# peterropac/Aegolius

Hardware: AMD Instinct MI355X
Metric: Mpoints/sec SDF eval, 1024^3 grid, 10-prim smooth-union tree (higher is better)
Workload: dtype f32

## Files before the change

aegolius_amd/_engine.py:

```python
import atexit
import contextlib
import ctypes
import importlib.util
import os
import sys
import threading

import numpy as np

_HERE = os.path.dirname(os.path.abspath(__file__))
LIB_PATH = os.path.join(_HERE, "libsdfk.so")

MODE_AUTO, MODE_INTERPRET, MODE_SPECIALIZED, MODE_NOCULL = 0, 1, 2, 3
(FLAVOUR_PLAIN_ARRAY, FLAVOUR_PLAIN_GRID, FLAVOUR_TILE_ARRAY, FLAVOUR_TILE_GRID, FLAVOUR_TILE_MASK, FLAVOUR_ROWS_ARRAY,
 FLAVOUR_ROWS_GRID, FLAVOUR_ROWS_MASK, FLAVOUR_ROWS2D_ARRAY, FLAVOUR_ROWS2D_GRID, FLAVOUR_RAYS) = range(11)
FLAVOUR_FLAGS = 0x100
FLAVOUR_XY = 0x200

_c = ctypes
_vp, _i64, _int, _sz = _c.c_void_p, _c.c_int64, _c.c_int, _c.c_size_t
_fp = _c.POINTER(_c.c_float)

SIGNATURES = {
    "sdfk_abi_version": (_int, []),
    "sdfk_device_count": (_int, []),
    "sdfk_last_error": (_c.c_char_p, []),
    "sdfk_program_create": (_vp, [_vp, _sz, _vp, _sz, _vp, _sz, _int]),
    "sdfk_program_destroy": (None, [_vp]),
    "sdfk_program_set_params": (_int, [_vp, _vp, _sz]),
    "sdfk_program_set_cull": (_int, [_vp, _vp, _sz, _vp]),
    "sdfk_program_source": (_c.c_char_p, [_vp]),
    "sdfk_program_compile_check": (_int, [_vp, _c.POINTER(_sz)]),
    "sdfk_program_chain_members": (_int, [_vp]),
    "sdfk_program_compile_flavour": (_int, [_vp, _int, _c.POINTER(_sz), _c.POINTER(_c.c_double)]),
    "sdfk_debug_compile_external": (_int, [_vp, _int, _c.POINTER(_sz)]),
    "sdfk_debug_jit_stats": (None, [_c.POINTER(_i64), _c.POINTER(_c.c_double)]),
    "sdfk_jit_drain": (None, []),
    "sdfk_jit_cancel": (None, []),
    "sdfk_debug_set_rtc_defs": (None, [_c.c_char_p]),
    "sdfk_eval_device": (_int, [_vp, _vp, _i64, _i64, _vp, _vp, _int]),
    "sdfk_eval_device_rows": (_int, [_vp, _vp, _i64, _i64, _i64, _vp, _vp, _int]),
    "sdfk_eval_device_rows2d": (_int, [_vp, _vp, _i64, _i64, _i64, _vp, _vp, _int]),
    "sdfk_eval_device_rows2d_xy": (_int, [_vp, _vp, _i64, _i64, _i64, _vp, _vp, _int]),
    "sdfk_debug_cells_stats": (None, [_int, _c.POINTER(_c.c_longlong)]),
    "sdfk_debug_rays_stats": (None, [_int, _c.POINTER(_c.c_longlong)]),
    "sdfk_eval_device_rows3d": (_int, [_vp, _vp, _i64, _i64, _i64, _i64, _i64, _vp, _vp, _int]),
    "sdfk_debug_row_masks": (_int, [_vp, _vp, _i64, _i64, _i64, _vp, _c.POINTER(_i64), _c.POINTER(_int), _vp]),
    "sdfk_eval_grid_sharded": (_int, [_vp, _vp, _i64, _vp, _i64, _vp, _i64, _int, _vp, _vp, _int]),
    "sdfk_eval_grid_sharded_device": (_int, [_vp, _vp, _i64, _vp, _i64, _vp, _i64, _int, _vp, _int, _vp, _int]),
    "sdfk_eval_device_aux": (_int, [_vp, _vp, _i64, _i64, _vp, _int, _i64, _vp, _vp, _int]),
    "sdfk_eval_grid_aux": (_int, [_vp, _vp, _i64, _vp, _i64, _vp, _i64, _i64, _i64, _vp, _int, _i64, _vp, _vp, _int]),
    "sdfk_field_min": (_int, [_vp, _i64, _c.POINTER(_c.c_float), _vp]),
    "sdfk_grid_box_average": (_int, [_vp, _i64, _i64, _i64, _int, _int, _int, _int, _vp, _vp]),
    "sdfk_grid_edge_detect": (_int, [_vp, _i64, _i64, _i64, _vp, _vp]),
    "sdfk_grid_signed": (_int, [_vp, _i64, _i64, _i64, _c.c_float, _int, _vp, _vp]),
    "sdfk_grid_boundary_mask": (_int, [_vp, _i64, _c.c_float, _vp, _vp]),
    "sdfk_grid_signed_slab": (_int, [_vp, _i64, _i64, _vp, _i64, _i64, _i64, _int, _vp, _vp]),
    "sdfk_eval_host": (_int, [_vp, _vp, _int, _i64, _i64, _vp, _int, _int]),
    "sdfk_eval_host_resident": (_int, [_vp, _vp, _int, _i64, _i64, _vp, _int, _int]),
    "sdfk_field_select_scratch": (_sz, [_i64]),
    "sdfk_field_select": (_int, [_vp, _i64, _c.c_float, _vp, _i64, _c.POINTER(_i64), _vp, _vp]),
    "sdfk_field_select_finish": (_int, [_i64, _i64, _vp, _i64, _vp, _vp]),
    "sdfk_field_gradient": (_int, [_vp, _i64, _i64, _i64, _int, _int, _vp, _i64, _vp]),
    "sdfk_field_crossings_2d": (_int, [_vp, _vp, _i64, _i64, _i64, _c.c_double, _c.c_double, _c.c_double, _vp, _vp]),
    "sdfk_lcwg_eval": (_int, [_int, _vp, _vp, _i64, _i64, _i64, _c.c_double, _c.c_double, _int, _c.c_double, _vp, _vp, _i64,
                              _vp]),
    "sdfk_lcwg_old_eval": (_int, [_int, _vp, _i64, _vp, _i64, _c.c_double, _c.c_double, _vp, _i64, _vp]),
    "sdfk_eval_select_scratch": (_sz, [_i64, _i64]),
    "sdfk_eval_device_select": (_int, [_vp, _vp, _i64, _i64, _i64, _int, _c.c_float, _vp, _i64, _c.POINTER(_i64), _vp, _vp, _int]),
    "sdfk_eval_grid_select": (_int, [_vp, _vp, _i64, _vp, _i64, _vp, _i64, _i64, _i64, _c.c_float, _vp, _i64, _c.POINTER(_i64),
                                     _vp, _vp, _int]),
    "sdfk_eval_select_finish": (_int, [_vp, _i64, _i64, _int, _i64, _vp, _i64, _vp, _vp]),
    "sdfk_vec_eval_device": (_int, [_vp, _int, _vp, _i64, _i64, _vp, _int, _i64, _int, _vp, _i64, _vp]),
    "sdfk_vec_set_interpret": (None, [_int]),
    "sdfk_vec_source": (_c.c_char_p, [_vp, _int, _int, _int]),
    "sdfk_vec_compile_check": (_int, [_vp, _int, _int, _int, _c.POINTER(_sz)]),
    "sdfk_vec_eval_host": (_int, [_vp, _int, _vp, _int, _i64, _vp, _i64, _vp, _i64, _vp, _i64, _vp, _int, _int, _vp, _int]),
    "sdfk_eval_grid": (_int, [_vp, _vp, _i64, _vp, _i64, _vp, _i64, _i64, _i64, _vp, _vp, _int]),
    "sdfk_eval_grid_host": (_int, [_vp, _vp, _i64, _vp, _i64, _vp, _i64, _i64, _i64, _vp, _int, _int]),
    "sdfk_set_default_mode": (None, [_int]),
    "sdfk_debug_brick_masks": (_int, [_vp, _vp, _i64, _i64, _vp, _vp]),
    "sdfk_linspace_f32": (_int, [_c.c_double, _c.c_double, _i64, _vp]),
    "sdfk_point_tree_build": (_i64, [_vp, _i64, _int, _vp, _i64, _vp, _vp, _vp]),
    "sdfk_grid_fill": (_int, [_vp, _i64, _vp, _i64, _vp, _i64, _vp, _i64, _i64, _i64, _vp]),
    "sdfk_set_device": (_int, [_int]),
    "sdfk_malloc": (_vp, [_sz]),
    "sdfk_free": (_int, [_vp]),
    "sdfk_memcpy_h2d": (_int, [_vp, _vp, _sz]),
    "sdfk_memcpy_d2h": (_int, [_vp, _vp, _sz]),
    "sdfk_memcpy_d2d": (_int, [_vp, _vp, _sz]),
    "sdfk_sync": (_int, [_vp]),
    "sdfk_event_create": (_vp, []),
    "sdfk_event_destroy": (_int, [_vp]),
    "sdfk_event_record": (_int, [_vp, _vp]),
    "sdfk_event_elapsed_ms": (_int, [_vp, _vp, _fp]),
    "sdfk_stream_probe": (_int, [_vp, _i64, _i64, _vp, _vp]),
    "sdfk_dual_has_rule": (_int, [_int]),
    "sdfk_program_jvp_check": (_int, [_vp, _c.POINTER(_int)]),
    "sdfk_eval_jvp_device": (_int, [_vp, _vp, _i64, _i64, _vp, _int, _int, _vp, _vp, _i64, _vp]),
    "sdfk_value_jvp_device": (_int, [_int, _vp, _vp, _vp, _i64, _vp, _vp, _vp]),
    "sdfk_program_vjp_check": (_int, [_vp, _c.POINTER(_int), _c.POINTER(_i64)]),
    "sdfk_vjp_limits": (_int, [_c.POINTER(_int), _c.POINTER(_int)]),
    "sdfk_eval_vjp_device": (_int, [_vp, _vp, _i64, _i64, _vp, _int, _int, _vp, _vp, _vp, _vp]),
    "sdfk_points_bin": (_int, [_vp, _i64, _i64, _vp, _i64, _i64, _i64, _vp, _vp]),
    "sdfk_points_extent": (_int, [_vp, _i64, _i64, _i64, _vp, _vp]),
    "sdfk_points_fill": (_int, [_vp, _i64, _i64, _i64, _int, _i64, _i64, _i64, _vp]),
    "sdfk_points_widen": (_int, [_vp, _i64, _int, _vp, _vp]),
    "sdfk_field_isosurface_scratch": (_sz, [_i64, _i64, _i64]),
    "sdfk_field_isosurface": (_int, [_vp, _vp, _i64, _vp, _i64, _vp, _i64, _c.c_float, _c.POINTER(_i64), _c.POINTER(_i64), _vp,
                                     _vp]),
    "sdfk_field_isosurface_finish": (_int, [_vp, _i64, _i64, _i64, _c.c_float, _i64, _i64, _vp, _i64, _vp, _i64, _int, _vp,
                                            _vp]),
    "sdfk_field_contour2d_scratch": (_sz, [_i64, _i64]),
    "sdfk_field_contour2d": (_int, [_vp, _vp, _i64, _vp, _i64, _c.c_float, _c.POINTER(_i64), _c.POINTER(_i64), _vp, _vp]),
    "sdfk_field_contour2d_finish": (_int, [_vp, _i64, _i64, _c.c_float, _i64, _i64, _vp, _i64, _vp, _i64, _int, _vp, _vp]),
    "sdfk_eval_grid_isosurface_scratch": (_sz, [_i64, _i64, _i64]),
    "sdfk_eval_grid_isosurface": (_int, [_vp, _vp, _i64, _vp, _i64, _vp, _i64, _c.c_float, _c.POINTER(_i64), _c.POINTER(_i64),
                                         _vp, _vp, _int]),
    "sdfk_eval_grid_isosurface_finish": (_int, [_vp, _vp, _i64, _vp, _i64, _vp, _i64, _c.c_float, _i64, _i64, _vp, _i64, _vp,
                                                _i64, _int, _vp, _vp, _int]),
    "sdfk_eval_grid_contour2d_scratch": (_sz, [_i64, _i64]),
    "sdfk_eval_grid_contour2d": (_int, [_vp, _vp, _i64, _vp, _i64, _c.c_float, _c.POINTER(_i64), _c.POINTER(_i64), _vp, _vp,
# ... 168 lines not shown

    def _filled(self, fill, *args):
        try:
            fill(*args)
        except BaseException:
            self.free()
            raise
        return self

    def free(self):
        _release(self, "ptr", "sdfk_free")

    def __enter__(self):
        return self

    def __exit__(self, *exc):
        self.free()

    def __del__(self):
        self.free()


class DeviceRows(DeviceBuffer):

    def __init__(self, rows, n, device=None, what=""):
        self.rows, self.n, self.stride = int(rows), int(n), row_stride(int(n))
        DeviceBuffer.__init__(self, self.rows * self.stride * 4, device, what)

    def offset(self, r):
        return 4 * r * self.stride

    def row(self, r):
        return self.at(self.offset(r), 4 * self.n)

    def row_ptr(self, r):
        return self.row(r).value

    def upload_rows(self, host):
        for r, line in enumerate(np.ascontiguousarray(host, dtype=np.float32)):
            self.upload(line, self.offset(r))

    def download_rows(self, count=None):
        out = np.empty((self.rows if count is None else count, self.n), dtype=np.float32)
        for r, line in enumerate(out):
            self.download(line, self.offset(r))
        return out


class Program:

    def __init__(self, code, params, tables, result_reg, cull_sites=None, cull_k=None):
        self.code = np.ascontiguousarray(code, dtype=np.uint32).reshape(-1, 2)
        self.params = np.ascontiguousarray(params, dtype=np.float32).ravel()
        self.tables = np.ascontiguousarray(tables, dtype=np.float32).ravel()
        self.result_reg = int(result_reg)
        self._h = lib().sdfk_program_create(_ptr(self.code), self.code.shape[0], _ptr(self.params), self.params.size,
                                            _ptr(self.tables), self.tables.size, self.result_reg)
        if not self._h:
            raise SdfkError("sdfk_program_create rejected the program: " + last_error())
        if cull_sites is not None and len(cull_sites):
            sites = np.ascontiguousarray(cull_sites, dtype=np.uint32).reshape(-1, 5)
            k = np.ascontiguousarray(cull_k, dtype=np.float32).ravel()
            check(lib().sdfk_program_set_cull(self._h, _ptr(sites), sites.shape[0], _ptr(k)), "sdfk_program_set_cull")

    @classmethod
    def from_lowered(cls, low, cull=True):
        if cull:
            return cls(low.code, low.params, low.tables, low.result_reg, low.cull_sites, low.cull_k)
        return cls(low.code, low.params, low.tables, low.result_reg)

    @property
    def handle(self):
        return self._h

    def set_params(self, params):
        p = np.ascontiguousarray(params, dtype=np.float32).ravel()
        check(lib().sdfk_program_set_params(self._h, _ptr(p), p.size), "sdfk_program_set_params")
        self.params = p

    def source(self):
        s = lib().sdfk_program_source(self._h)
        return s.decode() if s else None

    @property
    def chain_members(self):
        return int(lib().sdfk_program_chain_members(self._h))

    def compile_check(self):
        n = _sz(0)
        check(lib().sdfk_program_compile_check(self._h, ctypes.byref(n)), "sdfk_program_compile_check")
        return n.value

    def compile_flavour(self, flavour):
        n, t = _sz(0), _c.c_double(0.0)
        check(lib().sdfk_program_compile_flavour(self._h, int(flavour), ctypes.byref(n), ctypes.byref(t)),
              "sdfk_program_compile_flavour")
        return n.value, t.value

    def eval_host(self, co, device=0, mode=MODE_AUTO):
        require_gpu()
        co = host_coords(co)
        n = co.shape[1]
        out = np.empty(n, dtype=np.float32)
        check(lib().sdfk_eval_host(self._h, _ptr(co), 0 if co.dtype == np.float32 else 1, n, n, _ptr(out), device,
                                   mode), "sdfk_eval_host")
        return out

    def eval_device(self, d_co, n, row_stride, d_out, stream=None, mode=MODE_AUTO, row_len=None, flat=False,
                    plane_rows=None, first_row_in_plane=0):
        if row_len and plane_rows and not flat:
            check(lib().sdfk_eval_device_rows3d(self._h, _vp(d_co), n, row_stride, int(row_len), int(plane_rows),
                                                int(first_row_in_plane), _vp(d_out), _vp(stream or 0), mode),
                  "sdfk_eval_device_rows3d")
            return
        if row_len and flat:
            check(lib().sdfk_eval_device_rows2d(self._h, _vp(d_co), n, row_stride, int(row_len), _vp(d_out),
                                                _vp(stream or 0), mode), "sdfk_eval_device_rows2d")
            return
        if row_len:
            check(lib().sdfk_eval_device_rows(self._h, _vp(d_co), n, row_stride, int(row_len), _vp(d_out),
                                              _vp(stream or 0), mode), "sdfk_eval_device_rows")
            return
        check(lib().sdfk_eval_device(self._h, _vp(d_co), n, row_stride, _vp(d_out), _vp(stream or 0), mode),
              "sdfk_eval_device")

    def eval_device_xy(self, d_xy, n, row_stride, d_out, stream=None, mode=MODE_AUTO, row_len=None):
        check(lib().sdfk_eval_device_rows2d_xy(self._h, _vp(d_xy), n, row_stride, int(row_len or 0), _vp(d_out),
                                               _vp(stream or 0), mode), "sdfk_eval_device_rows2d_xy")

    def eval_grid(self, axes, start, count, d_out, stream=None, mode=MODE_AUTO):
        _, tab = axis_args(axes)
        check(lib().sdfk_eval_grid(self._h, *tab, start, count, _vp(d_out), _vp(stream or 0), mode), "sdfk_eval_grid")

    def _select(self, n, first, device, row_len=0, mode=MODE_AUTO):
        require_gpu()
        L = lib()
        check(L.sdfk_set_device(int(device)), "sdfk_set_device")

        def finish(m, d_index, d_scratch):
            check(L.sdfk_eval_select_finish(self._h, n, int(row_len), mode, m, d_index, m, d_scratch, None),
                  "sdfk_eval_select_finish")
        return _select(L.sdfk_eval_select_scratch(n, int(row_len)), first, finish)

    def select_grid(self, axes, threshold=0.0, start=0, count=None, device=0, mode=MODE_AUTO):
        ax, tab = axis_args(axes)
        total = ax[0].size * ax[1].size * ax[2].size
        count = total - start if count is None else count

        def first(d_scratch, m):
            check(lib().sdfk_eval_grid_select(self._h, *tab, start, count, float(threshold), None, 0, m, d_scratch, None,
                                              mode), "sdfk_eval_grid_select")
        grow = ax[2].size if ax[2].size > 1 else ax[1].size
        return self._select(count, first, device, row_len=grow if start % grow == 0 and count % grow == 0 else 0, mode=mode)

    def mesh_grid(self, axes, level, device=0, mode=MODE_AUTO, timings=None):
        require_gpu()
        check(lib().sdfk_set_device(int(device)), "sdfk_set_device")
        ax, tab = axis_args(axes)
        if len(ax) not in (2, 3):
            raise ValueError("mesh_grid: two or three axis tables")
        lead = (self._h,) + tab
        return extract_mesh("sdfk_eval_grid", [a.size for a in ax], level, lead, lead, (mode,), timings)

    def select_host(self, co, threshold=0.0, device=0, mode=MODE_AUTO):
        require_gpu()
        co32 = host_coords(co, np.float32)
# ... 280 lines not shown
```

aegolius_amd/csrc/sdfk.hip:

```cpp
#include <hip/hip_runtime.h>
#include <hip/hiprtc.h>

#include <chrono>
#include <algorithm>
#include <atomic>
#include <cmath>
#include <condition_variable>
#include <cstdio>
#include <cstdlib>
#include <cstring>
#include <deque>
#include <functional>
#include <map>
#include <memory>
#include <mutex>
#include <thread>
#include <string>
#include <vector>
#include <dirent.h>
#include <dlfcn.h>
#include <fcntl.h>
#include <signal.h>
#include <spawn.h>
#include <sys/wait.h>
// ... 93 lines not shown
    const unsigned lane_off = sdfk_tx() * 4;
    if (block_base + lane_off >= n) return;
    V3 p[4];
    sdfk_load<4>(src, block_base, lane_off, p);
    float v[4] = {p[0].x + p[0].y + p[0].z, p[1].x + p[1].y + p[1].z, p[2].x + p[2].y + p[2].z,
                  p[3].x + p[3].y + p[3].z};
    sdfk_store<4>(out, block_base + lane_off, v);
}

__global__ __launch_bounds__(SDFK_BLOCK) void sdfk_gridfill_kernel(SrcGrid src, long long n, float* __restrict__ co,
                                                                  long long stride) {
    const long long block_base = (long long)sdfk_bx() * (SDFK_BLOCK * 4);
    const unsigned lane_off = sdfk_tx() * 4;
    const long long i = block_base + lane_off;
    if (i >= n) return;
    V3 p[4];
    sdfk_load<4>(src, block_base, lane_off, p);
#pragma unroll
    for (int v = 0; v < 4; ++v) {
        if (i + v < n) {
            co[i + v] = p[v].x;
            co[stride + i + v] = p[v].y;
            co[2 * stride + i + v] = p[v].z;
        }
    }
}

static thread_local std::string g_err;
static int g_default_mode = SDFK_MODE_AUTO;

static int fail(int code, const std::string& msg) {
    g_err = msg;
    return code;
}
#define HIPCHK(expr)                                                                              \
    do {                                                                                          \
        hipError_t e_ = (expr);                                                                   \
        if (e_ != hipSuccess) {                                                                   \
            (void)hipGetLastError();  \
            return fail(-100 - (int)e_, std::string(#expr) + ": " + hipGetErrorString(e_));       \
        }                                                                                         \
    } while (0)

struct CellScratch {
    char* buf = nullptr;
    size_t bytes = 0;
};
struct DevState {
    uint2* d_code = nullptr;
    float* d_params = nullptr;
    float* d_tables = nullptr;
    unsigned long long params_version = 0;
    std::map<hipStream_t, CellScratch> cells;
};

struct CodeObject {
    std::mutex mu;
    std::condition_variable cv;
    int state = 0;
    std::vector<char> co;
    std::string error;
    std::string disk_path;
    double build_seconds = 0.0;
    std::chrono::steady_clock::time_point failed_at;
};
struct SpecModule {
    std::mutex mu;
    bool loaded = false, failed = false;
    hipModule_t mod = nullptr;
    hipFunction_t fn[4] = {nullptr, nullptr, nullptr, nullptr};
    std::string error;
};

struct sdfk_program {
    std::vector<uint32_t> code;
    std::vector<float> params, tables;
    int result_reg = 0;
    bool interp_ok = true;
    bool interp_small = false;
    int n_aux = 0;
    unsigned long long params_version = 1;
    std::string key;
    std::string source;
    std::vector<sdfk_cullsite> sites;
    std::vector<sdfk_cullsite> sites_all;
    bool chain_mode = false;
    int chain_members = 0;
    std::mutex mu;
    std::map<int, DevState> dev;
};

static std::mutex g_code_mu;
static std::map<std::string, std::shared_ptr<CodeObject>> g_code;
static std::map<std::pair<int, std::string>, std::shared_ptr<SpecModule>> g_mods;

extern "C" int sdfk_abi_version(void) { return SDFK_ABI_VERSION; }

extern "C" int sdfk_device_count(void) {
    int n = 0;
    if (hipGetDeviceCount(&n) != hipSuccess) {
        (void)hipGetLastError();
        return 0;
    }
    return n;
}

extern "C" const char* sdfk_last_error(void) { return g_err.c_str(); }
#define SDFK_MASK_SITES 512
extern "C" void sdfk_set_default_mode(int mode) { g_default_mode = mode; }

static int table_rows_ok(const sdfk_program* p, int op, const float* P, std::string* why) {
    auto bad = [&](const char* m) {
        *why = m;
        return 0;
    };
    long long cnt = (long long)P[0], off = (long long)P[1];
    if (op == SDFK_OP_P_POLYSIGN && P[0] == -1.0f) cnt = 1;
    else if (!(P[0] >= 0.0f) || (float)cnt != P[0]) return bad("table count/offset not integral");
    if (!(P[1] >= 0.0f) || (float)off != P[1]) return bad("table count/offset not integral");
    long long nt = (long long)p->tables.size();
    long long row = 0;
    switch (op) {
        case SDFK_OP_P_SEGLINE3: row = 7; break;
        case SDFK_OP_P_NEAREST3: row = 3; break;
        case SDFK_OP_P_SEGLINE2: row = 5; break;
        case SDFK_OP_P_NEAREST2: row = 2; break;
        case SDFK_OP_P_SHAPESIGN: row = 6; break;
        case SDFK_OP_CURVEINST: row = (P[2] != 0.0f) ? 12 : 3; break;
        case SDFK_OP_CURVEINSTT:
        case SDFK_OP_P_NEARTREE: {
            if (cnt < 1) return bad("point tree without root boxes");
            if (op == SDFK_OP_P_NEARTREE && P[2] != 2.0f && P[2] != 3.0f) return bad("point tree dimension must be 2 or 3");
            if (off + 8 * cnt > nt) return bad("point tree: root boxes out of range");
            const float* t = p->tables.data() + off;
            const long long room = nt - off;
            auto kids = [&](const float* box, long long width, long long* first, long long* n) {
                const float ff = box[6], fn = box[7];
                *first = (long long)ff;
                *n = (long long)fn;
                return ff >= 0.0f && fn >= 1.0f && (float)*first == ff && (float)*n == fn && *first + width * *n <= room;
            };
            for (long long r = 0; r < cnt; ++r) {
                long long mfirst, nm;
                if (!kids(t + 8 * r, 8, &mfirst, &nm)) return bad("point tree: middle boxes out of range");
                for (long long i = 0; i < nm; ++i) {
                    long long first, nl;
                    if (!kids(t + mfirst + 8 * i, 8, &first, &nl)) return bad("point tree: leaf boxes out of range");
                    for (long long l = 0; l < nl; ++l) {
                        long long pfirst, pcount;
                        if (!kids(t + first + 8 * l, 3, &pfirst, &pcount)) return bad("point tree: points out of range");
                        if (op == SDFK_OP_CURVEINSTT) {
                            const long long base = (long long)P[4], rows = (long long)P[3], ids = (long long)P[5];
                            const long long stride = (P[2] != 0.0f) ? 12 : 3;
                            if (!(P[3] >= 0.0f) || !(P[4] >= 0.0f) || !(P[5] >= 0.0f) || (float)base != P[4] || (float)rows != P[3] ||
                                (float)ids != P[5] || pfirst < base || (pfirst - base) % 3 != 0 ||
                                ids + (pfirst - base) / 3 + pcount > nt)
                                return bad("instancing tree: original indices out of range");
                            for (long long q = 0; q < pcount; ++q) {
                                const float of = p->tables[(size_t)(ids + (pfirst - base) / 3 + q)];
                                const long long o = (long long)of;
                                if (!(of >= 0.0f) || (float)o != of || rows + (o + 1) * stride > nt)
                                    return bad("instancing tree: instance row out of range");
                            }
                        }
                    }
                }
// ... 168 lines not shown
    for (size_t j = hi + 1; j < n; ++j) {
        instr_fields(p, j, &op, &a, &b, &c);
        const int kind = g_ops[op].kind;
        if (kind == SDFK_KIND_C_C || kind == SDFK_KIND_V_C) {
            if (wc[b]) return false;
        } else if (kind == SDFK_KIND_V_V) {
            if (wv[b]) return false;
        } else {
            const bool is_comb = (j == comb);
            if (wv[b] && !(is_comb && b == result_vreg)) return false;
            if (wv[c] && !(is_comb && c == result_vreg)) return false;
        }
        (kind == SDFK_KIND_C_C ? wc : wv)[a] = 0;
    }
    return !wv[(unsigned)p->result_reg];
}

static bool is_cullable_op(unsigned op) {
    return op == SDFK_OP_VMIN || op == SDFK_OP_VMAX || op == SDFK_OP_VSUBTRACT || op == SDFK_OP_SMIN2 ||
           op == SDFK_OP_SMIN3 || op == SDFK_OP_SMAX3 || op == SDFK_OP_SSUB3;
}

extern "C" int sdfk_program_set_cull(sdfk_program* p, const uint32_t* rows, size_t n_sites, const float* k) {
    if (!p) return fail(-1, "null program");
    if (n_sites > 32767) return fail(-2, "sdfk_program_set_cull: at most 32767 sites");
    if (n_sites && (!rows || !k)) return fail(-1, "sdfk_program_set_cull: null arrays");
    std::lock_guard<std::mutex> lk(p->mu);
    if (!p->source.empty() || !p->dev.empty())
        return fail(-2, "sdfk_program_set_cull: must be called before the program is first used");
    if (p->n_aux > 0) n_sites = 0;
    const size_t n = p->code.size() / 2;
    std::vector<sdfk_cullsite> sites;
    for (size_t i = 0; i < n_sites; ++i) {
        sdfk_cullsite t{rows[5 * i], rows[5 * i + 1], rows[5 * i + 2], rows[5 * i + 3], rows[5 * i + 4], k[i], 0, 0};
        if (!(t.comb < n && t.a0 <= t.a1 && t.a1 + 1 == t.b0 && t.b0 <= t.b1 && t.b1 + 1 == t.comb))
            return fail(-2, "sdfk_program_set_cull: malformed site ranges");
        if (!(t.k >= 0.0f) || !std::isfinite(t.k)) return fail(-2, "sdfk_program_set_cull: bad Lipschitz sum");
        unsigned op, a, b, c;
        instr_fields(p, t.comb, &op, &a, &b, &c);
        if (!is_cullable_op(op)) return fail(-2, "sdfk_program_set_cull: site is not at a min/max-type combiner");
        if (i && rows[5 * i] <= rows[5 * (i - 1)]) return fail(-2, "sdfk_program_set_cull: sites must be sorted");
        for (const sdfk_cullsite& u : sites) {
            const bool disjoint = u.comb < t.a0;
            const bool nested = u.a0 >= t.a0 && (u.comb <= t.a1 || (u.a0 >= t.b0 && u.comb <= t.b1));
            if (!disjoint && !nested) return fail(-2, "sdfk_program_set_cull: sites overlap without nesting");
        }
        t.skip_a_ok = range_skippable(p, t.a0, t.a1, t.comb, b) ? 1 : 0;
        t.skip_b_ok = range_skippable(p, t.b0, t.b1, t.comb, c) ? 1 : 0;
        sites.push_back(t);
    }
    p->sites_all = sites;
    if (sites.size() > SDFK_MASK_SITES) {
        std::vector<size_t> order(sites.size());
        for (size_t i = 0; i < order.size(); ++i) order[i] = i;
        std::stable_sort(order.begin(), order.end(), [&](size_t x, size_t y) {
            return (sites[x].a1 - sites[x].a0) + (sites[x].b1 - sites[x].b0) > (sites[y].a1 - sites[y].a0) + (sites[y].b1 - sites[y].b0);
        });
        order.resize(SDFK_MASK_SITES);
        std::sort(order.begin(), order.end());
        std::vector<sdfk_cullsite> widest;
        for (size_t i : order) widest.push_back(sites[i]);
        sites.swap(widest);
    }
    p->sites = sites;
    p->chain_members = sdfk_chain_mode(g_ops, SDFK_OP_COUNT, p->code.data(), p->code.size() / 2, p->result_reg, p->sites_all);
    p->chain_mode = p->chain_members > 0;
    p->key.append("|cull");
    for (const sdfk_cullsite& t : p->sites_all) {
        p->key.append(reinterpret_cast<const char*>(&t), sizeof t);
    }
    return 0;
}

extern "C" const char* sdfk_program_source(sdfk_program* p) {
    if (!p) return nullptr;
    std::lock_guard<std::mutex> lk(p->mu);
    if (p->source.empty())
        p->source = sdfk_generate_source(g_ops, SDFK_OP_COUNT, p->code.data(), p->code.size() / 2, p->result_reg,
                                         p->sites, SDFK_FL_ALL, &p->sites_all);
    return p->source.c_str();
}

static std::atomic<int> g_twaves_override{0}, g_rwbricks_override{0};
static int tile_waves() {
    static int v = [] { const char* e = getenv("SDFK_TWAVES"); int t = e ? atoi(e) : 4; return (t >= 1 && t <= 16) ? t : 4; }();
    const int o = g_twaves_override.load();
    return o ? o : v;
}
static int tile_wbricks() {
    static int v = [] {
        const char* e = getenv("SDFK_WBRICKS");
        int t = e ? atoi(e) : 4;
        if (t < 1 || t > 32) t = 4;
        return t;
    }();
    return v;
}
static int tile_points() { return tile_waves() * tile_wbricks() * 128; }
static std::atomic<int> g_rwaves_override{0};
static int rows_waves(const sdfk_program*) {
    if (const int o = g_rwaves_override.load()) return o;
    return 4;
}
static int rows_wbricks(const sdfk_program* p);
static long long big_program_limit() {
    static const long long v = [] {
        const char* e = getenv("SDFK_BIG_PROGRAM");
        const long long t = e ? atoll(e) : 300;
        return t > 0 ? t : 300;
    }();
    return v;
}
static int rows_geo(const sdfk_program* p) {
    const bool big = p && !p->chain_mode && (long long)(p->code.size() / 2) > big_program_limit();
    return rows_wbricks(p) | (rows_waves(p) << 4) | (big ? 1 << 16 : 0);
}
static int rows_wbricks(const sdfk_program* p) {
    static int forced = [] { const char* e = getenv("SDFK_RWBRICKS"); int t = e ? atoi(e) : 0; return (t >= 1 && t <= 16) ? t : 0; }();
    if (const int o = g_rwbricks_override.load()) return o;
    if (forced) return forced;
    if (p && p->chain_mode) return p->chain_members <= 64 ? 2 : 1;
    return 2;
}
struct RowGeom {
    unsigned L, nchunk, nbricks;
    long long R;
    long long row0;
    int yrows;
    unsigned prow, seg0, nb0, bpp;
    unsigned inv_nchunk, inv_bpp;
};
static bool rows_geometry(long long n, long long row_len, RowGeom* g, long long plane_rows = 0, long long plane_phase = 0,
                          bool planes_on = false) {
    if (row_len < 32 || row_len > 0x7fffffffLL || n <= 0 || n % row_len != 0) return false;
    const long long R = n / row_len, brows = 16;
    const long long nchunk = (row_len % 32 == 0) ? row_len / 32 : (row_len + 62) / 32;
    long long prow = plane_rows, seg0 = 0;
    static const bool plane_blocks = [] { const char* e = getenv("SDFK_PLANE_BLOCKS"); return e && e[0] == '1'; }();
    if (!(plane_blocks || planes_on) || prow <= 0 || prow >= R || prow > 0x7fffffffLL) {
        prow = R > 0x7fffffffLL ? 0 : R;
        if (prow == 0) return false;
    } else if (plane_phase > 0) {
        seg0 = std::min(R, (prow - plane_phase % prow) % prow);
    }
    const long long nb0 = (seg0 + brows - 1) / brows, bpp = (prow + brows - 1) / brows;
    const long long planes = (R - seg0 + prow - 1) / prow;
    const long long nb = nchunk * (nb0 + planes * bpp);
    if (nb > 0x7fffffffLL - 1024) return false;
    g->L = (unsigned)row_len;
    g->nchunk = (unsigned)nchunk;
    g->nbricks = (unsigned)nb;
    g->R = R;
    g->row0 = 0;
    g->yrows = 0;
    g->prow = (unsigned)prow;
    g->seg0 = (unsigned)seg0;
    g->nb0 = (unsigned)nb0;
    g->bpp = (unsigned)bpp;
    g->inv_nchunk = (unsigned)std::min<unsigned long long>(0xffffffffull, (1ull << 32) / (unsigned long long)nchunk);
    g->inv_bpp = (unsigned)std::min<unsigned long long>(0xffffffffull, (1ull << 32) / (unsigned long long)bpp);
    return true;
}
static int tile_threads() { return 64 * tile_waves(); }
static std::string rtc_cache_dir() {
    static const std::string dir = [] {
        std::string d;
        if (const char* e = getenv("SDFK_CACHE_DIR")) {
            d = e;
            if (d.empty() || d == "off" || d == "0") return std::string();
        } else if (const char* x = getenv("XDG_CACHE_HOME"); x && *x) {
            d = std::string(x) + "/sdfk";
        } else if (const char* h = getenv("HOME"); h && *h) {
            (void)mkdir((std::string(h) + "/.cache").c_str(), 0700);
            d = std::string(h) + "/.cache/sdfk";
        } else {
            return std::string();
        }
        (void)mkdir(d.c_str(), 0700);
        return d;
    }();
    return dir;
}
static std::string rtc_cache_path(const std::string& src, const std::string& opts) {
    const std::string dir = rtc_cache_dir();
    if (dir.empty()) return std::string();
    int major = 0, minor = 0;
    (void)hiprtcVersion(&major, &minor);
    unsigned long long h = 1469598103934665603ull;
    auto mix = [&](const std::string& t) {
        for (unsigned char c : t) {
            h ^= c;
            h *= 1099511628211ull;
        }
    };
    mix(src);
    mix(opts);
    mix(std::to_string(major) + "." + std::to_string(minor) + "/abi" + std::to_string(SDFK_ABI_VERSION));
    char name[96];
    snprintf(name, sizeof name, "/sdfk-%016llx-%zu.co", h, src.size());
    return dir + name;
}
static const unsigned long long kCacheMagic = 0x53444643'4f424a31ull;
static unsigned long long fnv1a(const char* p, size_t n) {
    unsigned long long h = 1469598103934665603ull;
    for (size_t i = 0; i < n; ++i) {
        h ^= (unsigned char)p[i];
        h *= 1099511628211ull;
    }
    return h;
}
static bool rtc_cache_read(const std::string& path, std::vector<char>* out) {
    if (path.empty()) return false;
    FILE* f = fopen(path.c_str(), "rb");
    if (!f) return false;
    bool ok = false;
    if (fseek(f, 0, SEEK_END) == 0) {
        const long size = ftell(f);
        if (size > 24 && fseek(f, 0, SEEK_SET) == 0) {
            out->resize((size_t)size);
            ok = fread(out->data(), 1, (size_t)size, f) == (size_t)size;
            if (ok) {
                unsigned long long tr[3];
                memcpy(tr, out->data() + size - 24, 24);
                ok = tr[0] == kCacheMagic && tr[1] == (unsigned long long)(size - 24) && tr[2] == fnv1a(out->data(), (size_t)size - 24);
                out->resize((size_t)size - 24);
            }
        }
    }
    fclose(f);
    if (!ok) {
        out->clear();
        (void)remove(path.c_str());
    } else {
        (void)utimes(path.c_str(), nullptr);
    }
    return ok;
}
static void rtc_cache_evict(const std::string& dir) {
    static const long long cap = [] {
        const char* e = getenv("SDFK_CACHE_MAX_MB");
        const long long v = e ? atoll(e) : 512;
        return (v > 0 ? v : 512) * (1ll << 20);
    }();
    DIR* d = opendir(dir.c_str());
    if (!d) return;
    std::vector<std::pair<long long, std::pair<std::string, long long>>> files;
    long long total = 0;
    while (dirent* e = readdir(d)) {
        const std::string name = e->d_name;
        if (name.compare(0, 5, "sdfk-") != 0 || name.compare(0, 9, "sdfk-rtc-") == 0) continue;
        struct stat st;
        const std::string path = dir + "/" + name;
        if (stat(path.c_str(), &st) != 0) continue;
        total += (long long)st.st_size;
        files.push_back({(long long)st.st_mtime, {path, (long long)st.st_size}});
    }
    closedir(d);
    if (total <= cap) return;
    std::sort(files.begin(), files.end());
    for (const auto& f : files) {
        if (total <= cap / 4 * 3) break;
        if (remove(f.second.first.c_str()) == 0) total -= f.second.second;
    }
}
static void rtc_cache_write(const std::string& path, const std::vector<char>& co) {
    if (path.empty() || co.empty()) return;
    const std::string tmp = path + ".tmp" + std::to_string((long long)getpid());
    FILE* f = fopen(tmp.c_str(), "wb");
    if (!f) return;
    const unsigned long long tr[3] = {kCacheMagic, (unsigned long long)co.size(), fnv1a(co.data(), co.size())};
    bool ok = fwrite(co.data(), 1, co.size(), f) == co.size() && fwrite(tr, 1, sizeof tr, f) == sizeof tr;
    ok = (fclose(f) == 0) && ok;
    if (!ok || rename(tmp.c_str(), path.c_str()) != 0) (void)remove(tmp.c_str());
    else rtc_cache_evict(rtc_cache_dir());
}

static std::mutex g_rtc_mu;
static std::mutex g_defs_mu;
static std::string g_rtc_defs = [] { const char* e = getenv("SDFK_RTC_DEFS"); return std::string(e ? e : ""); }();
extern "C" void sdfk_debug_set_rtc_defs(const char* defs) {
    std::lock_guard<std::mutex> lk(g_defs_mu);
    std::string rest;
    int tw = 0, rwb = 0, rwv = 0;
    const std::string all = defs ? defs : "";
    size_t pos = 0;
    while (pos < all.size()) {
        size_t sp = all.find(' ', pos);
        if (sp == std::string::npos) sp = all.size();
        const std::string tok = all.substr(pos, sp - pos);
        if (tok.compare(0, 14, "-DSDFK_TWAVES=") == 0) tw = atoi(tok.c_str() + 14);
        else if (tok.compare(0, 16, "-DSDFK_RWBRICKS=") == 0) rwb = atoi(tok.c_str() + 16);
        else if (tok.compare(0, 14, "-DSDFK_RWAVES=") == 0) rwv = atoi(tok.c_str() + 14);
        else if (!tok.empty()) rest += tok + " ";
        pos = sp + 1;
    }
    g_twaves_override = (tw >= 1 && tw <= 16) ? tw : 0;
    g_rwbricks_override = (rwb >= 1 && rwb <= 15) ? rwb : 0;
    g_rwaves_override = (rwv >= 1 && rwv <= 16) ? rwv : 0;
    g_rtc_defs = rest;
}
static std::vector<std::string> rtc_options(int geo) {
    const int rwb = geo & 15, rwaves = ((geo >> 4) & 0xff) ? ((geo >> 4) & 0xff) : 4;
    const bool big = (geo >> 16) & 1;
    const char* opt = getenv("SDFK_RTC_OPT");
    std::vector<std::string> o = {"--offload-arch=gfx950", (opt && opt[0] == '-') ? opt : "-O3", "-ffp-contract=off", "-std=c++17",
                                  "-fno-honor-nans", "-mno-amdgpu-ieee",
                                  "-DSDFK_TWAVES=" + std::to_string(tile_waves()), "-DSDFK_WBRICKS=" + std::to_string(tile_wbricks()),
                                  "-DSDFK_RWBRICKS=" + std::to_string(rwb), "-DSDFK_RWAVES=" + std::to_string(rwaves)};
    if (big) {
        o.push_back("-mllvm");
        o.push_back("-disable-cgp");
        o.push_back("-mllvm");
        o.push_back("-disable-vector-combine");
    }
    if (const char* extra = getenv("SDFK_RTC_EXTRA")) {
        std::string e = extra;
        size_t q = 0;
        while (q < e.size()) {
            size_t sp = e.find(' ', q);
            if (sp == std::string::npos) sp = e.size();
            if (sp > q) o.push_back(e.substr(q, sp - q));
            q = sp + 1;
        }
    }
    std::string all;
    {
        std::lock_guard<std::mutex> lk(g_defs_mu);
        all = g_rtc_defs;
    }
    size_t pos = 0;
    while (pos < all.size()) {
        size_t sp = all.find(' ', pos);
        if (sp == std::string::npos) sp = all.size();
        if (sp > pos && all.compare(pos, 2, "-D") == 0) o.push_back(all.substr(pos, sp - pos));
        pos = sp + 1;
    }
    return o;
}
static std::string rtc_option_key(int rwb) {
    std::string k;
    for (const std::string& o : rtc_options(rwb)) k += o + " ";
    return k;
}
static int rtc_compile_uncached(const std::string& src, std::vector<char>* out, std::string* log, int rwb) {
    hiprtcProgram prog = nullptr;
    if (hiprtcCreateProgram(&prog, src.c_str(), "sdfk_spec.hip", 0, nullptr, nullptr) != HIPRTC_SUCCESS) {
        *log = "hiprtcCreateProgram failed";
        return -1;
    }
    const std::vector<std::string> o = rtc_options(rwb);
    std::vector<const char*> opts;
    for (const std::string& x : o) opts.push_back(x.c_str());
    hiprtcResult r = hiprtcCompileProgram(prog, (int)opts.size(), opts.data());
    size_t ls = 0;
    hiprtcGetProgramLogSize(prog, &ls);
    if (ls > 1) {
        log->resize(ls);
        hiprtcGetProgramLog(prog, &(*log)[0]);
    }
    if (r != HIPRTC_SUCCESS) {
        *log = std::string("hiprtc: ") + hiprtcGetErrorString(r) + "\n" + *log;
        hiprtcDestroyProgram(&prog);
        return -1;
    }
    size_t cs = 0;
    hiprtcGetCodeSize(prog, &cs);
    out->resize(cs);
    hiprtcGetCode(prog, out->data());
    hiprtcDestroyProgram(&prog);
    return 0;
}
extern char** environ;
static std::string rtc_helper_path() {
    static const std::string path = [] {
        if (const char* e = getenv("SDFK_RTC_HELPER")) return std::string(strcmp(e, "off") && strcmp(e, "0") ? e : "");
        Dl_info info;
        if (!dladdr((void*)&sdfk_abi_version, &info) || !info.dli_fname) return std::string();
        std::string p = info.dli_fname;
        const size_t slash = p.rfind('/');
        p = (slash == std::string::npos ? std::string(".") : p.substr(0, slash)) + "/sdfk_rtc_helper";
        return access(p.c_str(), X_OK) == 0 ? p : std::string();
// ... 176 lines not shown
        std::unique_lock<std::mutex> lk(mu);
        cv.wait(lk, [this] { return jobs.empty() && busy == 0; });
    }
    void drop_queued() {
        std::lock_guard<std::mutex> lk(mu);
        jobs.clear();
        cv.notify_all();
    }
    ~BuildWorker() {
        {
            std::lock_guard<std::mutex> lk(mu);
            stop = true;
            cv.notify_all();
        }
        for (std::thread& t : threads)
            if (t.joinable()) t.join();
    }
};
static BuildWorker g_builds;
extern "C" void sdfk_jit_drain(void) { g_builds.drain(); }
extern "C" void sdfk_jit_cancel(void) {
    g_cancel_builds.store(true);
    g_builds.drop_queued();
    g_builds.drain();
}
static std::atomic<long long> g_compile_count{0};
static std::atomic<long long> g_compile_micros{0};
extern "C" void sdfk_debug_jit_stats(int64_t* builds, double* seconds) {
    if (builds) *builds = g_compile_count.load();
    if (seconds) *seconds = (double)g_compile_micros.load() * 1e-6;
}

static std::shared_ptr<CodeObject> code_entry(const std::string& key) {
    std::lock_guard<std::mutex> lk(g_code_mu);
    std::shared_ptr<CodeObject>& e = g_code[key];
    if (!e) e = std::make_shared<CodeObject>();
    return e;
}
static void code_build(const std::shared_ptr<CodeObject>& e, const std::string& src, int rwb, bool external = false) {
    const auto t0 = std::chrono::steady_clock::now();
    std::vector<char> co;
    std::string log;
    bool from_disk = false;
    std::string disk_path;
    const int rc = rtc_compile(src, &co, &log, rwb, &from_disk, &disk_path, external);
    const double dt = std::chrono::duration<double>(std::chrono::steady_clock::now() - t0).count();
    if (!from_disk) {
        g_compile_count++;
        g_compile_micros += (long long)(dt * 1e6);
    }
    std::lock_guard<std::mutex> lk(e->mu);
    e->build_seconds = dt;
    if (rc == 0) {
        e->co.swap(co);
        e->disk_path = disk_path;
        e->state = 2;
    } else {
        e->error = log;
        e->state = 3;
        e->failed_at = std::chrono::steady_clock::now();
    }
    e->cv.notify_all();
}
template <typename MakeSource>
static std::shared_ptr<CodeObject> code_get(const std::string& key, MakeSource make_source, int rwb, bool wait) {
    std::shared_ptr<CodeObject> e = code_entry(key);
    std::unique_lock<std::mutex> lk(e->mu);
    if (e->state == 3 && std::chrono::steady_clock::now() - e->failed_at > std::chrono::seconds(30)) e->state = 0;
    if (e->state == 0) {
        e->state = 1;
        lk.unlock();
        const std::string src = make_source();
        if (wait || !rtc_helper_available()) {
            code_build(e, src, rwb);
        } else {
            g_builds.post([e, src, rwb] { code_build(e, src, rwb, true); });
        }
        return e;
    }
    if (wait) e->cv.wait(lk, [&] { return e->state != 1; });
    return e;
}
static std::string flavour_key(const sdfk_program* p, int flavour, int rwb, int with_flags = 0) {
    return p->key + "|f" + std::to_string(flavour) + ((with_flags & 1) ? "s" : "") + ((with_flags & 2) ? "x" : "") + "|" + rtc_option_key(rwb);
}
static std::string flavour_source(const sdfk_program* p, int flavour, int with_flags = 0) {
    return std::string((with_flags & 1) ? "#define SDFK_FLAGS 1\n" : "") + ((with_flags & 2) ? "#define SDFK_XY 1\n" : "") +
           sdfk_generate_source(g_ops, SDFK_OP_COUNT, p->code.data(), p->code.size() / 2, p->result_reg, p->sites, flavour,
                                &p->sites_all);
}

extern "C" int sdfk_program_chain_members(const sdfk_program* p) {
    return p && p->chain_mode ? p->chain_members : 0;
}
extern "C" int sdfk_program_compile_check(sdfk_program* p, size_t* code_size) {
    if (!p) return fail(-1, "null program");
    size_t total = 0;
    const int rwb = rows_geo(p);
    for (int f = 0; f < SDFK_FL_COUNT; ++f) {
        if (f == SDFK_FL_RAYS) continue;
        if (p->sites.empty() && f != SDFK_FL_PLAIN_ARRAY && f != SDFK_FL_PLAIN_GRID) continue;
        if (p->chain_mode && (f == SDFK_FL_TILE_ARRAY || f == SDFK_FL_TILE_GRID || f == SDFK_FL_TILE_MASK || f == SDFK_FL_ROWS_MASK)) continue;
        std::shared_ptr<CodeObject> e = code_get(flavour_key(p, f, rwb), [&] { return flavour_source(p, f); }, rwb, true);
        if (e->state != 2) return fail(-3, e->error);
        total += e->co.size();
    }
    if (code_size) *code_size = total;
    return 0;
}
extern "C" int sdfk_program_compile_flavour(sdfk_program* p, int flavour, size_t* code_size, double* seconds) {
    if (!p) return fail(-1, "null program");
    int with_flags = 0;
    if (flavour >= 0 && (flavour & SDFK_FLAVOUR_FLAGS)) with_flags |= 1;
    if (flavour >= 0 && (flavour & SDFK_FLAVOUR_XY)) with_flags |= 2;
    if (flavour >= 0) flavour &= ~(SDFK_FLAVOUR_FLAGS | SDFK_FLAVOUR_XY);
    if (flavour < 0 || flavour >= SDFK_FL_COUNT) return fail(-1, "sdfk_program_compile_flavour: unknown flavour");
    if (p->sites.empty() && flavour != SDFK_FL_PLAIN_ARRAY && flavour != SDFK_FL_PLAIN_GRID && flavour != SDFK_FL_RAYS)
        return fail(-2, "sdfk_program_compile_flavour: the program has no cull sites");
    if (with_flags && flavour == SDFK_FL_RAYS)
        return fail(-2, "sdfk_program_compile_flavour: the ray flavour has no flag-writing or two-row build");
    if ((with_flags & 2) && flavour != SDFK_FL_PLAIN_ARRAY && flavour != SDFK_FL_ROWS2D_ARRAY)
        return fail(-2, "sdfk_program_compile_flavour: two-row coordinates exist for the plain and the flat row-block array kernels");
    if ((with_flags & 1) && (flavour == SDFK_FL_TILE_ARRAY || flavour == SDFK_FL_TILE_GRID || flavour == SDFK_FL_TILE_MASK ||
                       flavour == SDFK_FL_ROWS_MASK))
        return fail(-2, "sdfk_program_compile_flavour: this flavour has no flag-writing build");
    const int rwb = rows_geo(p);
    const auto t0 = std::chrono::steady_clock::now();
    std::shared_ptr<CodeObject> e =
        code_get(flavour_key(p, flavour, rwb, with_flags), [&] { return flavour_source(p, flavour, with_flags); }, rwb, true);
    if (e->state != 2) return fail(-3, e->error);
    if (code_size) *code_size = e->co.size();
    if (seconds) *seconds = std::chrono::duration<double>(std::chrono::steady_clock::now() - t0).count();
    return 0;
}

extern "C" int sdfk_debug_compile_external(sdfk_program* p, int flavour, size_t* code_size) {
    if (!p) return fail(-1, "null program");
    if (flavour < 0 || flavour >= SDFK_FL_COUNT) return fail(-1, "sdfk_debug_compile_external: unknown flavour");
    if (p->sites.empty() && flavour != SDFK_FL_PLAIN_ARRAY && flavour != SDFK_FL_PLAIN_GRID && flavour != SDFK_FL_RAYS)
        return fail(-2, "sdfk_debug_compile_external: the program has no cull sites");
    if (!rtc_helper_available()) return fail(-9, "sdfk_rtc_helper is not next to libsdfk.so (or hiprtc cannot be located)");
    std::vector<char> co;
    std::string log;
    if (rtc_compile_external(flavour_source(p, flavour), &co, &log, rows_geo(p)) != 0) return fail(-3, log);
    if (code_size) *code_size = co.size();
    return 0;
}

static std::shared_ptr<SpecModule> get_module(sdfk_program* p, int device, int flavour, bool wait, std::string* err,
                                              int with_flags = 0) {
    const int rwb = rows_geo(p);
    const std::string key = flavour_key(p, flavour, rwb, with_flags);
    std::shared_ptr<SpecModule> m;
    {
        std::lock_guard<std::mutex> lk(g_code_mu);
        std::shared_ptr<SpecModule>& slot = g_mods[std::make_pair(device, key)];
        if (!slot) slot = std::make_shared<SpecModule>();
        m = slot;
    }
    std::lock_guard<std::mutex> lk(m->mu);
    if (m->loaded) return m;
    for (int attempt = 0;; ++attempt) {
        std::shared_ptr<CodeObject> e;
        {
            std::lock_guard<std::mutex> ce(g_code_mu);
            auto it = g_code.find(key);
            if (it != g_code.end()) e = it->second;
        }
        int state = 0;
        if (e) {
            std::lock_guard<std::mutex> el(e->mu);
            state = e->state;
        }
        if (state != 2) {
            e = code_get(key, [&] { return flavour_source(p, flavour, with_flags); }, rwb, wait);
            std::lock_guard<std::mutex> el(e->mu);
            state = e->state;
        }
        if (state == 1) return nullptr;
        if (state != 2) {
            std::lock_guard<std::mutex> el(e->mu);
            *err = e->error;
            m->failed = true;
            m->error = e->error;
            return m;
        }
        hipError_t he;
        {
            std::lock_guard<std::mutex> rl(g_rtc_mu);
            he = hipModuleLoadData(&m->mod, e->co.data());
        }
        for (int i = 0; i < 2 && he == hipSuccess; ++i)
            if (kFlavourFn[flavour][i]) he = hipModuleGetFunction(&m->fn[i], m->mod, kFlavourFn[flavour][i]);
        if (he == hipSuccess && p->chain_mode && !kFlavourFn[flavour][1]) {
            const bool grid_fl = flavour == SDFK_FL_ROWS_GRID || flavour == SDFK_FL_ROWS2D_GRID;
            if (hipModuleGetFunction(&m->fn[1], m->mod, grid_fl ? "sdfk_spec_cellsg" : "sdfk_spec_cells") != hipSuccess) {
                m->fn[1] = nullptr;
                (void)hipGetLastError();
            }
        }
        if (he == hipSuccess && flavour == SDFK_FL_RAYS) {
            if (hipModuleGetFunction(&m->fn[2], m->mod, "sdfk_spec_rays_cull") != hipSuccess ||
                hipModuleGetFunction(&m->fn[3], m->mod, "sdfk_spec_raycam_cull") != hipSuccess) {
                m->fn[2] = m->fn[3] = nullptr;
                (void)hipGetLastError();
            }
        }
        if (he == hipSuccess) break;
        bool retry = false;
        {
            std::lock_guard<std::mutex> el(e->mu);
            if (attempt == 0 && e->state == 2 && !e->disk_path.empty()) {
                (void)remove(e->disk_path.c_str());
                fprintf(stderr, "[sdfk] cached code object %s does not load (%s): rebuilding\n", e->disk_path.c_str(),
                        hipGetErrorString(he));
                e->disk_path.clear();
// ... 126 lines not shown
                 o_head = (o_cspan + 8 * nc + 63) & ~(size_t)63, o_pool = o_head + 2 * 64 * shards, total = o_pool + 4 * cap + 64;
    CellScratch* cs;
    {
        std::lock_guard<std::mutex> lk(p->mu);
        cs = &d->cells[stream];
    }
    if (cs->bytes < total) {
        if (cs->buf) {
            HIPCHK(hipStreamSynchronize(stream));
            (void)hipFree(cs->buf);
            cs->buf = nullptr;
            cs->bytes = 0;
        }
        if (hipMalloc(&cs->buf, total + total / 4) != hipSuccess) { (void)hipGetLastError(); return 0; }
        cs->bytes = total + total / 4;
    }
    char* b = cs->buf;
    HIPCHK(hipMemsetAsync(b + o_head, 0, 2 * 64 * shards, stream));
    CellPassArg cp{};
    cp.cand = b + o_pool;
    if (coarse) {
        cp.lv = crs; cp.parent = CellLevelH{}; cp.sph = b + o_csph; cp.span = b + o_cspan; cp.psph = nullptr; cp.pspan = nullptr;
        cp.ncells = (unsigned)nc; cp.inflate = 1.3f;
        cp.head = reinterpret_cast<unsigned*>(b + o_head);
        cp.base = 0u; cp.shard_cap = (unsigned)cshard;
        std::vector<void*> args = {(void*)&prm, (void*)&tab};
        for (int i = 0; i < n_src; ++i) args.push_back(src[i]);
        RowGeom g2 = rg;
        args.push_back(&g2);
        args.push_back(&cp);
        HIPCHK(hipModuleLaunchKernel(cells_fn, (unsigned)((nc + 3) / 4), 1, 1, 256, 1, 1, 0, stream, args.data(), nullptr));
    }
    cp.lv = fine; cp.parent = coarse ? crs : CellLevelH{}; cp.sph = b + o_fsph; cp.span = b + o_fspan;
    cp.psph = coarse ? b + o_csph : nullptr; cp.pspan = coarse ? b + o_cspan : nullptr;
    cp.ncells = (unsigned)nf; cp.inflate = 1.0f;
    cp.head = reinterpret_cast<unsigned*>(b + o_head + 64 * shards);
    cp.base = (unsigned)(shards * cshard); cp.shard_cap = (unsigned)fshard;
    {
        std::vector<void*> args = {(void*)&prm, (void*)&tab};
        for (int i = 0; i < n_src; ++i) args.push_back(src[i]);
        RowGeom g2 = rg;
        args.push_back(&g2);
        args.push_back(&cp);
        HIPCHK(hipModuleLaunchKernel(cells_fn, (unsigned)((nf + 3) / 4), 1, 1, 256, 1, 1, 0, stream, args.data(), nullptr));
    }
    static const bool trace = [] { const char* e = getenv("SDFK_CELLS_TRACE"); return e && e[0] == '1'; }();
    if (trace || g_cells_stats_on.load()) {
        HIPCHK(hipStreamSynchronize(stream));
        std::vector<uint2> sp(nf);
        unsigned head = 0;
        HIPCHK(hipMemcpy(sp.data(), b + o_fspan, 8 * nf, hipMemcpyDeviceToHost));
        {
            std::vector<unsigned> heads(2 * 16 * shards);
            HIPCHK(hipMemcpy(heads.data(), b + o_head, 2 * 64 * shards, hipMemcpyDeviceToHost));
            for (size_t i = 0; i < heads.size(); i += 16) head += heads[i];
        }
        unsigned long long sum = 0, all = 0, empty = 0, mx = 0;
        for (const uint2& x : sp) {
            if (x.y == 0xffffffffu) ++all;
            else { sum += x.y; mx = std::max<unsigned long long>(mx, x.y); if (x.y == 0) ++empty; }
        }
        {
            std::lock_guard<std::mutex> lk(g_cells_stats_mu);
            g_cells_stats[0] = (long long)nf; g_cells_stats[1] = (long long)nc; g_cells_stats[2] = (long long)head;
            g_cells_stats[3] = (long long)cap; g_cells_stats[4] = (long long)sum; g_cells_stats[5] = (long long)mx;
            g_cells_stats[6] = (long long)all; g_cells_stats[7] = (long long)empty;
        }
        if (trace) fprintf(stderr, "[sdfk cells] %d members: fine %ux%ux%u = %llu cells (2^%u planes x 2^%u blocks x 2^%u windows), coarse %llu; pool %u of %llu entries; "
                "fine lists: mean %.1f max %llu, %llu without a list, %llu empty\n", p->chain_members, fine.ncx, fine.ncy, fine.ncz, nf, fine.lx, fine.ly, fine.lz, nc,
                head, cap, (double)sum / (double)std::max<unsigned long long>(1, nf - all - empty), mx, all, empty);
    }
    out->lv = fine;
    out->sph = b + o_fsph;
    out->span = b + o_fspan;
    out->cand = b + o_pool;
    out->enabled = 1u;
    out->ncells = (unsigned)nf;
    return 0;
}

static int run(sdfk_program* p, const SrcArray* arr, const SrcGrid* grid, long long n, float* d_out, void* stream_,
               int mode, bool vec_ok, long long row_len = 0, const float* aux = nullptr, long long aux_stride = 0,
               bool flat = false, long long plane_rows = 0, long long plane_phase = 0, unsigned* d_flags = nullptr,
               unsigned thr_key = 0, bool xy = false) {
    if (!p) return fail(-1, "null program");
    if (n < 0) return fail(-1, "negative point count");
    if (p->n_aux > 0 && (!aux || aux_stride < n))
        return fail(-1, "this program reads auxiliary fields (staged evaluation): use sdfk_eval_device_aux / sdfk_eval_grid_aux");
    if (n == 0) return 0;
    if (mode == SDFK_MODE_AUTO) mode = g_default_mode;
    if (d_flags && (mode == SDFK_MODE_AUTO || mode == SDFK_MODE_INTERPRET)) mode = SDFK_MODE_SPECIALIZED;
    if (xy) {
        if (!arr || p->n_aux > 0) return fail(-1, "two-row coordinates: array source, no auxiliary fields");
        if (mode == SDFK_MODE_AUTO || mode == SDFK_MODE_INTERPRET) mode = SDFK_MODE_SPECIALIZED;
    }
    hipStream_t stream = (hipStream_t)stream_;
    int device = 0;
    HIPCHK(hipGetDevice(&device));
    DevState* d = nullptr;
    int rc = ensure_resident(p, device, stream, &d);
    if (rc) return rc;

    long long n4 = vec_ok ? (n / 4) * 4 : 0;
    long long tail = n - n4;

    static const long long spec_limit = [] {
        const char* e = getenv("SDFK_SPECIALIZE_LIMIT");
        const long long v = e ? atoll(e) : 1200;
        return v > 0 ? v : 1200;
    }();
    static const long long rows_limit = [] {
        const char* e = getenv("SDFK_ROWS_LIMIT");
        const long long v = e ? atoll(e) : 1200;
        return v > 0 ? v : 1200;
    }();
    if (mode == SDFK_MODE_AUTO && (long long)(p->code.size() / 2) > spec_limit && p->interp_ok && !p->chain_mode && !d_flags)
        mode = SDFK_MODE_INTERPRET;

    RowGeom rg;
    int flavour = arr ? SDFK_FL_PLAIN_ARRAY : SDFK_FL_PLAIN_GRID;
    const long long grow = grid ? (grid->n2 > 1 ? (long long)grid->n2 : (long long)grid->n1) : 0;
    if (!p->sites.empty() && mode != SDFK_MODE_NOCULL && mode != SDFK_MODE_INTERPRET) {
        if (arr && rows_geometry(n, row_len, &rg, (flat || d_flags) ? 0 : plane_rows, plane_phase, p->chain_mode))
            flavour = (flat || xy) ? SDFK_FL_ROWS2D_ARRAY : SDFK_FL_ROWS_ARRAY;
        else if (arr && vec_ok && !p->chain_mode && !d_flags && !xy) flavour = SDFK_FL_TILE_ARRAY;
        else if (grid && grid->start % grow == 0 &&
                 rows_geometry(n, grow, &rg, (grid->n2 > 1 && !d_flags) ? (long long)grid->n1 : 0,
                               grid->n2 > 1 ? (grid->start / grow) % (long long)grid->n1 : 0, p->chain_mode))
            flavour = grid->n2 > 1 ? SDFK_FL_ROWS_GRID : SDFK_FL_ROWS2D_GRID;
        else if (grid && vec_ok && !p->chain_mode && !d_flags) flavour = SDFK_FL_TILE_GRID;
        if (!p->chain_mode && (long long)(p->code.size() / 2) > rows_limit &&
            (flavour == SDFK_FL_ROWS_ARRAY || flavour == SDFK_FL_ROWS2D_ARRAY || flavour == SDFK_FL_ROWS_GRID || flavour == SDFK_FL_ROWS2D_GRID)) {
            const bool is_arr = arr != nullptr;
            if (vec_ok && !d_flags && !xy) flavour = is_arr ? SDFK_FL_TILE_ARRAY : SDFK_FL_TILE_GRID;
            else if (!d_flags) flavour = is_arr ? SDFK_FL_PLAIN_ARRAY : SDFK_FL_PLAIN_GRID;
        }
    }
    std::shared_ptr<SpecModule> sk;
    if (mode != SDFK_MODE_INTERPRET) {
        static const bool async_jit = [] { const char* e = getenv("SDFK_ASYNC_JIT"); return !(e && e[0] == '0'); }();
        const bool wait = mode != SDFK_MODE_AUTO || !p->interp_ok || !async_jit;
        std::string err;
        sk = get_module(p, device, flavour, wait, &err, (d_flags ? 1 : 0) | (xy ? 2 : 0));
        if (sk && sk->failed) {
            if (mode == SDFK_MODE_SPECIALIZED || !p->interp_ok)
                return fail(-3, "specialised kernel unavailable: " + err);
            static bool warned = false;
            if (!warned) {
                fprintf(stderr, "[sdfk] hiprtc specialisation failed, using the interpreter kernel: %s\n", err.c_str());
                warned = true;
            }
            sk.reset();
        }
    }
    if (!sk && !p->interp_ok)
        return fail(-4, "program needs more registers than the interpreter kernel has (use the specialised mode)");

    const float* prm = d->d_params;
    const float* tab = d->d_tables;
    if (sk) {
        if (flavour == SDFK_FL_ROWS_ARRAY || flavour == SDFK_FL_ROWS_GRID || flavour == SDFK_FL_ROWS2D_ARRAY ||
            flavour == SDFK_FL_ROWS2D_GRID) {
            const unsigned per_tile = (unsigned)(rows_waves(p) * rows_wbricks(p));
            const unsigned tiles = ((rg.nbricks + per_tile - 1) / per_tile + 127u) & ~127u;
            const unsigned rthreads = 64u * (unsigned)rows_waves(p);
            CellsArg cells{};
            const bool with_cells = p->chain_mode && sk->fn[1] != nullptr;
            if (arr) {
                const float* co = arr->co;
                long long stride = arr->stride;
                if (with_cells) {
                    void* src[] = {&co, &stride};
                    rc = prepare_cells(p, d, sk->fn[1], rg, src, 2, prm, tab, stream, &cells);
                    if (rc) return rc;
                }
                void* args[] = {&prm, &tab, &co, &stride, &rg, &d_out, &d_flags, &thr_key, &cells};
                HIPCHK(hipModuleLaunchKernel(sk->fn[0], tiles, 1, 1, rthreads, 1, 1, 0, stream, args, nullptr));
            } else {
                SrcGrid g = *grid;
                rg.row0 = grid->start / grow;
                rg.yrows = grid->n2 > 1 ? 0 : 1;
                if (with_cells) {
                    void* src[] = {&g};
                    rc = prepare_cells(p, d, sk->fn[1], rg, src, 1, prm, tab, stream, &cells);
                    if (rc) return rc;
                }
                void* args[] = {&prm, &tab, &g, &rg, &d_out, &d_flags, &thr_key, &cells};
                HIPCHK(hipModuleLaunchKernel(sk->fn[0], tiles, 1, 1, rthreads, 1, 1, 0, stream, args, nullptr));
            }
            return 0;
        }
        if (flavour == SDFK_FL_TILE_ARRAY || flavour == SDFK_FL_TILE_GRID) {
            const unsigned tiles = (unsigned)((n + tile_points() - 1) / tile_points());
            if (arr) {
                const float* co = arr->co;
                long long stride = arr->stride;
                void* args[] = {&prm, &tab, &co, &stride, &n, &d_out};
                HIPCHK(hipModuleLaunchKernel(sk->fn[0], tiles, 1, 1, tile_threads(), 1, 1, 0, stream, args, nullptr));
            } else {
                SrcGrid g = *grid;
                void* args[] = {&prm, &tab, &g, &n, &d_out};
                HIPCHK(hipModuleLaunchKernel(sk->fn[0], tiles, 1, 1, tile_threads(), 1, 1, 0, stream, args, nullptr));
            }
            return 0;
        }
        if (arr) {
            const float* co = arr->co;
            long long stride = arr->stride;
            if (n4) {
                long long off = 0;
                void* args[] = {&prm, &tab, &co, &stride, &off, &n4, &d_out, &aux, &aux_stride, &d_flags, &thr_key};
                HIPCHK(hipModuleLaunchKernel(sk->fn[0], blocks_for(n4, 4), 1, 1, SDFK_BLOCK, 1, 1, 0, stream, args,
                                             nullptr));
            }
            if (tail) {
                long long off = n4;
                void* args[] = {&prm, &tab, &co, &stride, &off, &tail, &d_out, &aux, &aux_stride, &d_flags, &thr_key};
                HIPCHK(hipModuleLaunchKernel(sk->fn[1], blocks_for(tail, 1), 1, 1, SDFK_BLOCK, 1, 1, 0, stream, args,
                                             nullptr));
            }
        } else {
            SrcGrid g = *grid;
            if (n4) {
                long long off = 0;
                void* args[] = {&prm, &tab, &g, &off, &n4, &d_out, &aux, &aux_stride, &d_flags, &thr_key};
                HIPCHK(hipModuleLaunchKernel(sk->fn[0], blocks_for(n4, 4), 1, 1, SDFK_BLOCK, 1, 1, 0, stream, args,
                                             nullptr));
            }
            if (tail) {
                long long off = n4;
                void* args[] = {&prm, &tab, &g, &off, &tail, &d_out, &aux, &aux_stride, &d_flags, &thr_key};
                HIPCHK(hipModuleLaunchKernel(sk->fn[1], blocks_for(tail, 1), 1, 1, SDFK_BLOCK, 1, 1, 0, stream, args,
                                             nullptr));
            }
        }
        return 0;
    }
    if (d_flags) return fail(-3, "fused selection needs the specialised kernels");
    const int n_instr = (int)(p->code.size() / 2);
    const long long zero = 0;
    auto launch = [&](auto src, int vec, long long off, long long cnt) {
        using SRC = decltype(src);
        const dim3 grid(blocks_for(cnt, vec)), block(SDFK_BLOCK);
#define SDFK_INTERP_GO(VEC, NC, NV) hipLaunchKernelGGL((sdfk_interp_kernel<VEC, NC, NV, SRC>), grid, block, 0, stream, d->d_code, \
                                                        n_instr, prm, tab, src, off, cnt, d_out, p->result_reg, aux, aux_stride)
        if (vec == 4) {
            if (p->interp_small) SDFK_INTERP_GO(4, SDFK_NC_SMALL, SDFK_NV_SMALL);
            else SDFK_INTERP_GO(4, SDFK_NC, SDFK_NV);
        } else {
            if (p->interp_small) SDFK_INTERP_GO(1, SDFK_NC_SMALL, SDFK_NV_SMALL);
            else SDFK_INTERP_GO(1, SDFK_NC, SDFK_NV);
        }
#undef SDFK_INTERP_GO
    };
    if (arr) {
        if (n4) launch(*arr, 4, zero, n4);
        if (tail) launch(*arr, 1, n4, tail);
    } else {
        if (n4) launch(*grid, 4, zero, n4);
        if (tail) launch(*grid, 1, n4, tail);
    }
    HIPCHK(hipGetLastError());
    return 0;
}

static bool aligned16(const void* p) { return (reinterpret_cast<uintptr_t>(p) & 15u) == 0; }

extern "C" int sdfk_eval_device(sdfk_program* p, const float* d_co, int64_t n, int64_t row_stride, float* d_out,
                                void* stream, int mode) {
    if (!d_co || !d_out) return fail(-1, "sdfk_eval_device: null device pointer");
// ... 52 lines not shown
extern "C" int sdfk_eval_device_aux(sdfk_program* p, const float* d_co, int64_t n, int64_t row_stride, const float* d_aux,
                                    int n_aux, int64_t aux_stride, float* d_out, void* stream, int mode) {
    if (!p || !d_co || !d_out) return fail(-1, "sdfk_eval_device_aux: null pointer");
    if (row_stride < n) return fail(-1, "sdfk_eval_device_aux: row stride smaller than the point count");
    if (n_aux < p->n_aux) return fail(-1, "sdfk_eval_device_aux: the program reads more auxiliary fields than were passed");
    SrcArray a = {d_co, (long long)row_stride};
    bool vec_ok = aligned16(d_co) && aligned16(d_out) && (row_stride % 4 == 0);
    return run(p, &a, nullptr, n, d_out, stream, mode, vec_ok, 0, d_aux, aux_stride);
}

extern "C" int sdfk_debug_row_masks(sdfk_program* p, const float* d_co, int64_t n, int64_t row_stride, int64_t row_len,
                                    uint64_t* d_masks, int64_t* n_bricks, int* brick_rows, void* stream_) {
    if (!p || !d_co) return fail(-1, "sdfk_debug_row_masks: null argument");
    if (p->sites.empty()) return fail(-2, "sdfk_debug_row_masks: program has no cull sites");
    if (p->chain_mode) return fail(-2, "sdfk_debug_row_masks: a chain-mode program keeps lists of surviving children, not mask words");
    RowGeom rg;
    if (row_stride < n || !rows_geometry(n, row_len, &rg))
        return fail(-1, "sdfk_debug_row_masks: the row-block kernel does not take this shape");
    if (n_bricks) *n_bricks = rg.nbricks;
    if (brick_rows) *brick_rows = 16;
    if (!d_masks) return 0;
    hipStream_t stream = (hipStream_t)stream_;
    int device = 0;
    HIPCHK(hipGetDevice(&device));
    DevState* d = nullptr;
    int rc = ensure_resident(p, device, stream, &d);
    if (rc) return rc;
    std::string err;
    std::shared_ptr<SpecModule> sk = get_module(p, device, SDFK_FL_ROWS_MASK, true, &err);
    if (!sk || sk->failed) return fail(-3, "specialised kernel unavailable: " + err);
    const float* prm = d->d_params;
    const float* tab = d->d_tables;
    long long stride = row_stride;
    void* args[] = {&prm, &tab, &d_co, &stride, &rg, &d_masks};
    const unsigned per_tile = (unsigned)(rows_waves(p) * rows_wbricks(p));
    HIPCHK(hipModuleLaunchKernel(sk->fn[0], (rg.nbricks + per_tile - 1) / per_tile, 1, 1, 64 * rows_waves(p), 1, 1, 0, stream,
                                 args, nullptr));
    return 0;
}

extern "C" int sdfk_debug_brick_masks(sdfk_program* p, const float* d_co, int64_t n, int64_t row_stride,
                                      uint64_t* d_masks, void* stream_) {
    if (!p || !d_co || !d_masks) return fail(-1, "sdfk_debug_brick_masks: null argument");
    if (!(aligned16(d_co) && row_stride % 4 == 0 && row_stride >= n && n > 0))
        return fail(-1, "sdfk_debug_brick_masks: needs 16-byte aligned rows");
    if (p->sites.empty()) return fail(-2, "sdfk_debug_brick_masks: program has no cull sites");
    if (p->chain_mode) return fail(-2, "sdfk_debug_brick_masks: chain-mode programs have no line-brick flavour");
    hipStream_t stream = (hipStream_t)stream_;
    int device = 0;
    HIPCHK(hipGetDevice(&device));
    DevState* d = nullptr;
    int rc = ensure_resident(p, device, stream, &d);
    if (rc) return rc;
    std::string err;
    std::shared_ptr<SpecModule> sk = get_module(p, device, SDFK_FL_TILE_MASK, true, &err);
    if (!sk || sk->failed) return fail(-3, "specialised kernel unavailable: " + err);
    const float* prm = d->d_params;
    const float* tab = d->d_tables;
    long long stride = row_stride, nn = n;
    void* args[] = {&prm, &tab, &d_co, &stride, &nn, &d_masks};
    HIPCHK(hipModuleLaunchKernel(sk->fn[0], (unsigned)((n + tile_points() - 1) / tile_points()), 1, 1, tile_threads(),
                                 1, 1, 0, stream, args, nullptr));
    return 0;
}

extern "C" int sdfk_linspace_f32(double lo, double hi, int64_t n, float* out) {
    if (n < 0 || (n > 0 && !out)) return fail(-1, "sdfk_linspace_f32: bad arguments");
    if (n == 0) return 0;
    if (n == 1) {
        out[0] = (float)lo;
        return 0;
    }
    const double div = (double)(n - 1);
    const double delta = hi - lo;
    const double step = delta / div;
    for (int64_t i = 0; i < n; ++i) {
        volatile double t = (step != 0.0) ? (double)i * step : ((double)i / div) * delta;
        out[i] = (float)(t + lo);
    }
    out[n - 1] = (float)hi;
    return 0;
}

struct AxisTables {
    float* d = nullptr;
    ~AxisTables() {
        if (d) (void)hipFree(d);
    }
};

static int upload_axes(const float* ax0, int64_t n0, const float* ax1, int64_t n1, const float* ax2, int64_t n2,
                       hipStream_t stream, AxisTables* t, SrcGrid* g, int64_t start) {
    if (!ax0 || !ax1 || !ax2 || n0 < 1 || n1 < 1 || n2 < 1) return fail(-1, "grid axes missing or empty");
    if (n1 > 0x7fffffff || n2 > 0x7fffffff) return fail(-1, "grid axis too long");
    HIPCHK(hipMalloc(&t->d, (size_t)(n0 + n1 + n2) * sizeof(float)));
    HIPCHK(hipMemcpyAsync(t->d, ax0, (size_t)n0 * sizeof(float), hipMemcpyHostToDevice, stream));
    HIPCHK(hipMemcpyAsync(t->d + n0, ax1, (size_t)n1 * sizeof(float), hipMemcpyHostToDevice, stream));
    HIPCHK(hipMemcpyAsync(t->d + n0 + n1, ax2, (size_t)n2 * sizeof(float), hipMemcpyHostToDevice, stream));
    g->ax0 = t->d;
    g->ax1 = t->d + n0;
    g->ax2 = t->d + n0 + n1;
    g->n1 = (unsigned)n1;
    g->n2 = (unsigned)n2;
    g->start = start;
    return 0;
}

extern "C" int sdfk_eval_grid(sdfk_program* p, const float* ax0, int64_t n0, const float* ax1, int64_t n1,
                              const float* ax2, int64_t n2, int64_t start, int64_t count, float* d_out, void* stream,
                              int mode) {
    if (!d_out) return fail(-1, "sdfk_eval_grid: null output");
    if (start < 0 || count < 0 || start + count > n0 * n1 * n2) return fail(-1, "sdfk_eval_grid: range outside the grid");
    AxisTables t;
    SrcGrid g;
    int rc = upload_axes(ax0, n0, ax1, n1, ax2, n2, (hipStream_t)stream, &t, &g, start);
    if (rc) return rc;
    rc = run(p, nullptr, &g, count, d_out, stream, mode, aligned16(d_out));
    if (rc) return rc;
    HIPCHK(hipStreamSynchronize((hipStream_t)stream));
    return 0;
}

extern "C" int sdfk_eval_grid_aux(sdfk_program* p, const float* ax0, int64_t n0, const float* ax1, int64_t n1,
                                  const float* ax2, int64_t n2, int64_t start, int64_t count, const float* d_aux, int n_aux,
                                  int64_t aux_stride, float* d_out, void* stream, int mode) {
    if (!p || !d_out) return fail(-1, "sdfk_eval_grid_aux: null pointer");
    if (start < 0 || count < 0 || start + count > n0 * n1 * n2) return fail(-1, "sdfk_eval_grid_aux: range outside the grid");
    if (n_aux < p->n_aux) return fail(-1, "sdfk_eval_grid_aux: the program reads more auxiliary fields than were passed");
    AxisTables t;
    SrcGrid g;
    int rc = upload_axes(ax0, n0, ax1, n1, ax2, n2, (hipStream_t)stream, &t, &g, start);
    if (rc) return rc;
    rc = run(p, nullptr, &g, count, d_out, stream, mode, aligned16(d_out), 0, d_aux, aux_stride);
    if (rc) return rc;
    HIPCHK(hipStreamSynchronize((hipStream_t)stream));
    return 0;
}

extern "C" int sdfk_eval_grid_host(sdfk_program* p, const float* ax0, int64_t n0, const float* ax1, int64_t n1,
                                   const float* ax2, int64_t n2, int64_t start, int64_t count, float* out, int device,
                                   int mode) {
    if (!p) return fail(-1, "null program");
    if (count < 0 || (count > 0 && !out)) return fail(-1, "sdfk_eval_grid_host: bad arguments");
    if (start < 0 || start + count > n0 * n1 * n2) return fail(-1, "sdfk_eval_grid_host: range outside the grid");
    if (count == 0) return 0;
    HIPCHK(hipSetDevice(device));
    int64_t chunk = std::min<int64_t>(count, (int64_t)1 << 27);
    const int64_t grow = n2 > 1 ? n2 : n1;
    if (start % grow == 0 && chunk > grow) chunk = chunk / grow * grow;
    float* d_out = nullptr;
    HIPCHK(hipMalloc(&d_out, (size_t)chunk * sizeof(float)));
    AxisTables t;
    SrcGrid g;
    int rc = upload_axes(ax0, n0, ax1, n1, ax2, n2, nullptr, &t, &g, start);
    for (int64_t s = 0; s < count && rc == 0; s += chunk) {
        const int64_t m = std::min(chunk, count - s);
        g.start = start + s;
        rc = run(p, nullptr, &g, m, d_out, nullptr, mode, true);
        if (rc == 0 && hipMemcpy(out + s, d_out, (size_t)m * sizeof(float), hipMemcpyDeviceToHost) != hipSuccess)
            rc = fail(-6, "sdfk_eval_grid_host: device-to-host copy failed");
    }
    (void)hipFree(d_out);
    return rc;
}

extern "C" int sdfk_eval_grid_sharded(sdfk_program* p, const float* ax0, int64_t n0, const float* ax1, int64_t n1,
                                      const float* ax2, int64_t n2, int n_shards, const int* devices, float* out,
                                      int mode) {
    if (!p || !out) return fail(-1, "sdfk_eval_grid_sharded: null argument");
    if (n_shards < 1 || n_shards > 64) return fail(-1, "sdfk_eval_grid_sharded: 1..64 shards");
    if (!ax0 || !ax1 || !ax2 || n0 < 1 || n1 < 1 || n2 < 1) return fail(-1, "grid axes missing or empty");
    int n_dev = 0;
    if (hipGetDeviceCount(&n_dev) != hipSuccess || n_dev < 1) return fail(-8, "sdfk_eval_grid_sharded: no HIP device");
    const int64_t total = n0 * n1 * n2, unit = n2 > 1 ? n2 : n1;
    const int64_t per = (total / unit / n_shards) * unit;
    std::vector<int> rc((size_t)n_shards, 0);
    std::vector<std::string> msg((size_t)n_shards);
    std::vector<std::thread> workers;
    for (int d = 0; d < n_shards; ++d) {
        const int dev = devices ? devices[d] : d % n_dev;
        if (dev < 0 || dev >= n_dev) return fail(-1, "sdfk_eval_grid_sharded: device index out of range");
    }
    for (int d = 0; d < n_shards; ++d) {
        const int dev = devices ? devices[d] : d % n_dev;
        const int64_t start = d * per, count = d < n_shards - 1 ? per : total - start;
        workers.emplace_back([=, &rc, &msg] {
            rc[(size_t)d] = count > 0 ? sdfk_eval_grid_host(p, ax0, n0, ax1, n1, ax2, n2, start, count, out + start, dev, mode) : 0;
            if (rc[(size_t)d]) msg[(size_t)d] = sdfk_last_error();
        });
    }
    for (std::thread& t : workers) t.join();
    for (int d = 0; d < n_shards; ++d)
        if (rc[(size_t)d]) return fail(rc[(size_t)d], "shard " + std::to_string(d) + ": " + msg[(size_t)d]);
    return 0;
}

extern "C" int sdfk_eval_grid_sharded_device(sdfk_program* p, const float* ax0, int64_t n0, const float* ax1, int64_t n1,
                                             const float* ax2, int64_t n2, int n_shards, const int* devices,
                                             int gather_device, float* d_full, int mode) {
    if (!p || !d_full) return fail(-1, "sdfk_eval_grid_sharded_device: null argument");
    if (n_shards < 1 || n_shards > 64) return fail(-1, "sdfk_eval_grid_sharded_device: 1..64 shards");
    if (!ax0 || !ax1 || !ax2 || n0 < 1 || n1 < 1 || n2 < 1) return fail(-1, "grid axes missing or empty");
    int n_dev = 0;
    if (hipGetDeviceCount(&n_dev) != hipSuccess || n_dev < 1) return fail(-8, "sdfk_eval_grid_sharded_device: no HIP device");
    if (gather_device < 0 || gather_device >= n_dev) return fail(-1, "sdfk_eval_grid_sharded_device: gather device out of range");
    for (int d = 0; d < n_shards; ++d) {
        const int dev = devices ? devices[d] : d % n_dev;
        if (dev < 0 || dev >= n_dev) return fail(-1, "sdfk_eval_grid_sharded_device: device index out of range");
    }
    const int64_t total = n0 * n1 * n2, unit = n2 > 1 ? n2 : n1;
    const int64_t per = (total / unit / n_shards) * unit;
    std::vector<int> rc((size_t)n_shards, 0);
    std::vector<std::string> msg((size_t)n_shards);
    std::vector<std::thread> workers;
    for (int d = 0; d < n_shards; ++d) {
        const int dev = devices ? devices[d] : d % n_dev;
        const int64_t start = d * per, count = d < n_shards - 1 ? per : total - start;
        workers.emplace_back([=, &rc, &msg] {
            auto shard = [&]() -> int {
                if (count <= 0) return 0;
                HIPCHK(hipSetDevice(dev));
                hipStream_t stream = nullptr;
                HIPCHK(hipStreamCreateWithFlags(&stream, hipStreamNonBlocking));
                static const bool force_copy = [] { const char* e = getenv("SDFK_FORCE_PEER_COPY"); return e && e[0] == '1'; }();
                const bool in_place = dev == gather_device && !force_copy;
                float* d_slab = in_place ? d_full + start : nullptr;
                int r = 0;
                if (!d_slab && hipMalloc(&d_slab, (size_t)count * sizeof(float)) != hipSuccess) r = fail(-5, "out of device memory for the slab");
                if (r == 0) r = sdfk_eval_grid(p, ax0, n0, ax1, n1, ax2, n2, start, count, d_slab, stream, mode);
                if (r == 0 && !in_place) {
                    if (hipMemcpyPeerAsync(d_full + start, gather_device, d_slab, dev, (size_t)count * sizeof(float), stream) != hipSuccess ||
                        hipStreamSynchronize(stream) != hipSuccess)
                        r = fail(-6, "peer copy of the slab failed");
                }
                if (!in_place && d_slab) (void)hipFree(d_slab);
                (void)hipStreamDestroy(stream);
                return r;
            };
            rc[(size_t)d] = shard();
            if (rc[(size_t)d]) msg[(size_t)d] = sdfk_last_error();
        });
// ... 298 lines not shown
```

aegolius_amd/csrc/sdfk_codegen.cpp:

```cpp
#include "sdfk_codegen.h"

#include <algorithm>
#include <cstdio>
#include <cstring>
#include <map>
#include <set>

#include "sdfk_embedded.inc"

std::string sdfk_vector_prelude() { return std::string(kEmbeddedDevice) + "\n" + kEmbeddedVecdev + "\n"; }

static const char kWrappers[] = R"SDFKW(
template <int VEC, typename SRC>
static __device__ __forceinline__ void sdfk_body(const float* __restrict__ PRM, const float* __restrict__ TAB,
                                                 const SRC& src, long long off, long long n,
                                                 float* __restrict__ out, const float* __restrict__ aux,
                                                 long long aux_stride, unsigned* __restrict__ flags, unsigned thr) {
    const long long block_base = (long long)sdfk_bx() * (SDFK_BLOCK * VEC);
    const unsigned lane_off = sdfk_tx() * VEC;
#ifdef SDFK_FLAGS                                              // the flag-writing build of this flavour (its own code object:
    {                                                          // carried as a run-time branch it cost the field kernels registers)
        const bool active = block_base + lane_off < n;
        unsigned nib = 0u;
        if (active) {
// ... 1594 lines not shown
#pragma unroll
    for (int bt = 0; bt < SDFK_CELL_NB; ++bt)
        if (64u * bt < cnt) total += (unsigned)__builtin_popcountll(__ballot(64u * bt + (unsigned)lane < cnt && !(ev[bt] - m >= thr0 + 1e-6f * fabsf(ev[bt]))));
#pragma unroll 4
    for (unsigned j0 = 64u * SDFK_CELL_NB; j0 < cnt; j0 += 64u) {
        const unsigned j = j0 + (unsigned)lane;
        bool run = false;
        if (j < cnt) {
            const float e = SDFK_CHAIN_SGN * sdfk_leaf_rec<float>(listed ? cp.cand[off + j] : sdfk_member_record(j), c, PRM, TAB);
            run = !(e - m >= thr0 + 1e-6f * fabsf(e));
        }
        total += (unsigned)__builtin_popcountll(__ballot(run));
    }
    // per microsecond and address), so the pool is cut into SDFK_POOL_SHARDS shards with a head each, dealt by cell index
    unsigned at = 0u;
    const unsigned shard = cell & (SDFK_POOL_SHARDS - 1u);
    if (lane == 0) at = atomicAdd(cp.head + 16u * shard, total);
    at = __shfl(at, 0);
    if (at > cp.shard_cap || total > cp.shard_cap - at) {       // the shard is full: bricks of this cell probe every member
        if (lane == 0) cp.span[cell] = make_uint2(0u, SDFK_ALL_ALIVE);
        return;
    }
    at += cp.base + shard * cp.shard_cap;
    unsigned n_out = 0u;
#pragma unroll
    for (int bt = 0; bt < SDFK_CELL_NB; ++bt)
        if (64u * bt < cnt) {
            const bool run = 64u * bt + (unsigned)lane < cnt && !(ev[bt] - m >= thr0 + 1e-6f * fabsf(ev[bt]));
            const unsigned long long bits = __ballot(run);
            if (run) cp.cand[at + n_out + (unsigned)__builtin_popcountll(bits & ((1ull << lane) - 1ull))] = rv[bt];
            n_out += (unsigned)__builtin_popcountll(bits);
        }
#pragma unroll 4
    for (unsigned j0 = 64u * SDFK_CELL_NB; j0 < cnt; j0 += 64u) {
        const unsigned j = j0 + (unsigned)lane;
        bool run = false;
        unsigned rec = 0u;
        if (j < cnt) {
            rec = listed ? cp.cand[off + j] : sdfk_member_record(j);
            const float e = SDFK_CHAIN_SGN * sdfk_leaf_rec<float>(rec, c, PRM, TAB);
            run = !(e - m >= thr0 + 1e-6f * fabsf(e));
        }
        const unsigned long long bits = __ballot(run);
        if (run) cp.cand[at + n_out + (unsigned)__builtin_popcountll(bits & ((1ull << lane) - 1ull))] = rec;
        n_out += (unsigned)__builtin_popcountll(bits);
    }
    if (lane == 0) cp.span[cell] = make_uint2(at, total);
}
#else
#define SDFK_CELLS_KARG
#endif
)SDFKR";
static const char kRowsArray[] = R"SDFKR(
extern "C" __global__ __launch_bounds__(64 * SDFK_RWAVES) SDFK_ROWS_ATTR void sdfk_spec_r(
    const float* __restrict__ PRM, const float* __restrict__ TAB, const float* __restrict__ co, long long stride,
    sdfk_rowgeom g, float* __restrict__ out, unsigned* __restrict__ flags, unsigned thr SDFK_CELLS_KARG) {
    const SrcArray s = {co, stride};
    sdfk_rows_kernel(PRM, TAB, s, g, out, flags, thr SDFK_CELLS_PASS);
}
#ifdef SDFK_CELLS
extern "C" __global__ __launch_bounds__(256) void sdfk_spec_cells(
    const float* __restrict__ PRM, const float* __restrict__ TAB, const float* __restrict__ co, long long stride,
    sdfk_rowgeom g, sdfk_cellpass cp) {
    const SrcArray s = {co, stride};
    sdfk_cells_kernel(PRM, TAB, s, g, cp);
}
#endif
)SDFKR";
static const char kRowsGrid[] = R"SDFKR(
// the same on a regular grid expanded from three per-axis tables (no coordinate array: 4 B/point); the slab
// starts at a row boundary and out[0] is its first point
extern "C" __global__ __launch_bounds__(64 * SDFK_RWAVES) void sdfk_spec_rg(
    const float* __restrict__ PRM, const float* __restrict__ TAB, SrcGrid s, sdfk_rowgeom g, float* __restrict__ out,
    unsigned* __restrict__ flags, unsigned thr SDFK_CELLS_KARG) {
    sdfk_rows_kernel(PRM, TAB, s, g, out, flags, thr SDFK_CELLS_PASS);
}
#ifdef SDFK_CELLS
extern "C" __global__ __launch_bounds__(256) void sdfk_spec_cellsg(
    const float* __restrict__ PRM, const float* __restrict__ TAB, SrcGrid s, sdfk_rowgeom g, sdfk_cellpass cp) {
    sdfk_cells_kernel(PRM, TAB, s, g, cp);
}
#endif
)SDFKR";
static const char kRowsMask[] = R"SDFKR(
// test aid: the skip masks (two 64-bit words per brick: sites 0-31, 32-63; bit 2k = first operand of site k
// skipped, bit 2k+1 = second) followed by the "uniform rows" flag in a third word
extern "C" __global__ __launch_bounds__(64 * SDFK_RWAVES) void sdfk_spec_rmask(
    const float* __restrict__ PRM, const float* __restrict__ TAB, const float* __restrict__ co, long long stride,
    sdfk_rowgeom g, unsigned long long* __restrict__ masks) {
    __shared__ __attribute__((aligned(16))) sdfk_rowmeta meta;
    const SrcArray s = {co, stride};
    unsigned rb, c;
    sdfk_rows_prepare(PRM, TAB, s, g, &meta, sdfk_bx(), rb, c);
    const unsigned q = sdfk_bx() * SDFK_RNBRICK + sdfk_tx();
    if (sdfk_tx() < SDFK_RNBRICK && q < g.nbricks) {
        masks[3ull * q] = meta.mask[0][sdfk_tx()];
        masks[3ull * q + 1] = meta.mask[1][sdfk_tx()];
        masks[3ull * q + 2] = meta.uniform[sdfk_tx()];
    }
}
)SDFKR";

namespace {

struct Gen {
    const sdfk_opinfo* ops;
    int n_ops;
    const uint32_t* code;
    size_t n_instr;
    const std::vector<sdfk_cullsite>* sites;
    std::string s;
    bool rows = false;

    std::vector<int> root_slot;
    int n_root = 0;
    void find_roots() {
        root_slot.assign(n_instr, -1);
        bool c0_intact = true;
        for (size_t i = 0; i < n_instr; ++i) {
            const uint32_t w = code[2 * i];
            const unsigned op = w & 255u, a = (w >> 8) & 255u, b = (w >> 16) & 255u;
            if ((int)op >= n_ops) continue;
            if (ops[op].kind != SDFK_KIND_C_C) continue;
            if (!strcmp(ops[op].name, "XFORM") && b == 0 && c0_intact && n_root < 64) root_slot[i] = n_root++;
            if (a == 0) c0_intact = false;
        }
    }

    void instr_x(size_t i, const char* indent, int mode) {
        const int r = root_slot.empty() ? -1 : root_slot[i];
        if (r < 0 || mode == 0 || (rows && mode == 1)) {
            instr(i, indent, rows && mode == 2);
            return;
        }
        char buf[1400];
        const uint32_t w = code[2 * i], poff = code[2 * i + 1];
        const unsigned a = (w >> 8) & 255u;
        if (rows) {
            snprintf(buf, sizeof buf,
                     "%sif constexpr (ZRUN) {\n"
                     "#ifdef SDFK_FLAT\n"
                     "%s  const V3T<float> bs = op_xform_base_x(X, PRM + %u);\n"
                     "%s  const V3P bp = {sp<f2>(bs.x), sp<f2>(bs.y), sp<f2>(bs.z)};\n"
                     "%s  SDFK_EACH C_%u[q] = op_xform_y(bp, C_0[q].y, PRM + %u);\n"
                     "#else\n"
                     "%s  const V3T<float> bs = op_xform_base(X, Y, PRM + %u);\n"
                     "%s  const V3P bp = {sp<f2>(bs.x), sp<f2>(bs.y), sp<f2>(bs.z)};\n"
                     "%s  SDFK_EACH C_%u[q] = op_xform_z(bp, C_0[q].z, PRM + %u);\n"
                     "#endif\n"
                     "%s} else { SDFK_EACH C_%u[q] = op_xform(C_0[q], PRM + %u, TAB, 0); }\n",
                     indent, indent, poff, indent, indent, a, poff, indent, poff, indent, indent, a, poff, indent, a, poff);
        } else if (mode == 1) {
            snprintf(buf, sizeof buf,
                     "%s{ const V3T<float> bs = op_xform_base(C_0.x, C_0.y, PRM + %u); bases[%d] = bs.x; bases[%d] = bs.y; "
                     "bases[%d] = bs.z;\n%s  C_%u = op_xform_z(bs, C_0.z, PRM + %u); }\n",
                     indent, poff, 3 * r, 3 * r + 1, 3 * r + 2, indent, a, poff);
        } else {
            snprintf(buf, sizeof buf,
                     "%sif constexpr (ZRUN) { const V3T<T> bs = {sp<T>(bases[%d]), sp<T>(bases[%d]), sp<T>(bases[%d])};\n"
                     "%s  C_%u = op_xform_z(bs, C_0.z, PRM + %u); }\n%selse C_%u = op_xform(C_0, PRM + %u, TAB, 0);\n",
                     indent, 3 * r, 3 * r + 1, 3 * r + 2, indent, a, poff, indent, a, poff);
        }
        s += buf;
    }

    void instr(size_t i, const char* indent) { instr(i, indent, false); }
// ... 837 lines not shown
                   "#define SDFK_SIMT 1\n#define SDFK_NSUB 1\n"
                   "#ifndef SDFK_CELLS_MIN_LEAVES\n#define SDFK_CELLS_MIN_LEAVES 64\n#endif\n"
                   "#if !defined(SDFK_NO_CELLS) && SDFK_NLEAF > SDFK_CELLS_MIN_LEAVES\n#define SDFK_CELLS 1\n#endif\n"
                   "#ifndef SDFK_LEAF_UNROLL\n#define SDFK_LEAF_UNROLL _Pragma(\"unroll 4\")\n#endif\n";
            g.s += kSimtGeometry;
            g.emit_probe_leaves(g.leaves.size() >= 128, true);
            g.s += kRowsKernel;
            if (all || flavour == SDFK_FL_ROWS_ARRAY || flavour == SDFK_FL_ROWS2D_ARRAY) g.s += kRowsArray;
            if (all || flavour == SDFK_FL_ROWS_GRID || flavour == SDFK_FL_ROWS2D_GRID) g.s += kRowsGrid;
        }
        return g.s;
    }
    if (plain) {
        g.s += "\ntemplate <typename T> static __device__ __forceinline__ T sdfk_point(V3T<T> C_0, "
               "const float* __restrict__ PRM, const float* __restrict__ TAB, const float* __restrict__ AUX, "
               "long long AUXS) {\n";
        g.declare("V3T<T>", "T", false);
        for (size_t i = 0; i < n_instr; ++i) g.instr(i, "    ");
        snprintf(buf, sizeof buf, "    return V_%d;\n}\n", result_reg);
        g.s += buf;
        g.s += kWrappers;
        if (all || flavour == SDFK_FL_PLAIN_ARRAY) g.s += kWrappersArray;
        if (all || flavour == SDFK_FL_PLAIN_GRID) g.s += kWrappersGrid;
    }
    if (tile || rowk) g.s += kWaveHelpers;
    if (tile) {
        std::vector<size_t> order(sites.size());
        for (size_t i = 0; i < order.size(); ++i) order[i] = i;
        std::stable_sort(order.begin(), order.end(), [&](size_t x, size_t y) {
            return sites[x].comb - sites[x].a0 > sites[y].comb - sites[y].a0;
        });
        order.resize(std::min<size_t>(order.size(), 31));
        std::sort(order.begin(), order.end());
        std::vector<sdfk_cullsite> flat;
        for (size_t i : order) flat.push_back(sites[i]);
        g.sites = &flat;
        g.find_roots();
        snprintf(buf, sizeof buf, "\n#define SDFK_NROOT %d\n", g.n_root > 0 ? g.n_root : 1);
        g.s += buf;
        g.emit_probe();
        g.emit_culled(result_reg);
        g.s += kTileKernel;
        if (all || flavour == SDFK_FL_TILE_ARRAY) g.s += kTileArray;
        if (all || flavour == SDFK_FL_TILE_GRID) g.s += kTileGrid;
        if (all || flavour == SDFK_FL_TILE_MASK) g.s += kTileMask;
        g.sites = &sites;
    }
    if (rowk) {
        g.rows = true;
        g.root_slot.clear();
        g.n_root = 0;
        g.find_roots();
        if (flat) g.s += "\n#define SDFK_FLAT 1\n";
        g.s += "\n#define SDFK_NP 4\n#define SDFK_EACH _Pragma(\"unroll\") for (int q = 0; q < SDFK_NP; ++q)\n";
        {
            char nm[64];
            snprintf(nm, sizeof nm, "#define SDFK_NMASK %zu\n", std::max<size_t>(2, (sites.size() + 31) / 32));
            g.s += nm;
        }
        g.s += "#ifndef SDFK_CHAIN_LOOP_MIN\n#define SDFK_CHAIN_LOOP_MIN 100000   // chains of at least this many sites run as a loop over the levels that survive\n#endif\n"
               "// the even bits of x, packed into the low 32 bits (wave-uniform: scalar unit)\n"
               "static __device__ __forceinline__ unsigned long long sdfk_even_bits(unsigned long long x) {\n"
               "    x &= 0x5555555555555555ull;\n"
               "    x = (x | (x >> 1)) & 0x3333333333333333ull;\n"
               "    x = (x | (x >> 2)) & 0x0f0f0f0f0f0f0f0full;\n"
               "    x = (x | (x >> 4)) & 0x00ff00ff00ff00ffull;\n"
               "    x = (x | (x >> 8)) & 0x0000ffff0000ffffull;\n"
               "    x = (x | (x >> 16)) & 0x00000000ffffffffull;\n"
               "    return x;\n}\n";
        g.simt = g.analyse_leaves();
        if (g.simt) {
            char def[160];
            snprintf(def, sizeof def, "\n#ifndef SDFK_NOSIMT\n#define SDFK_SIMT 1\n#endif\n#define SDFK_NLEAF %zu\n", g.leaves.size());
            g.s += def;
            g.s += kSimtGeometry;
            g.emit_groups();
            g.emit_probe_leaves();
            g.emit_probe_fold();
        }
        g.emit_probe();
        g.emit_rows_culled(result_reg);
        g.s += kRowsKernel;
        if (all || flavour == SDFK_FL_ROWS_ARRAY || flavour == SDFK_FL_ROWS2D_ARRAY) g.s += kRowsArray;
        if (all || flavour == SDFK_FL_ROWS_GRID || flavour == SDFK_FL_ROWS2D_GRID) g.s += kRowsGrid;
        if (all || flavour == SDFK_FL_ROWS_MASK) g.s += kRowsMask;
    }
    return g.s;
}
```

aegolius_amd/csrc/sdfk_fieldops.inc:

```

#include "sdfk_vecdev.h"

#define SDFK_SEL_THREADS 256
#define SDFK_SEL_ITERS 8
#define SDFK_SEL_TILE (SDFK_SEL_THREADS * 4 * SDFK_SEL_ITERS)
#ifndef SDFK_SEL_TPW
#define SDFK_SEL_TPW 4
#endif

static __device__ __forceinline__ int sdfk_wave_inclusive(int v, int lane) {
    for (int d = 1; d < 64; d <<= 1) {
        const int t = __shfl_up(v, d, 64);
        if (lane >= d) v += t;
    }
    return v;
}

static __device__ __forceinline__ unsigned sdfk_sel_flags(const float* __restrict__ f, long long i, long long n, unsigned thr) {
    if (i + 4 <= n) {
        const sdfk_f4 v = __builtin_nontemporal_load(reinterpret_cast<const sdfk_f4*>(f + i));
        return (sdfk_sel_key(v[0]) <= thr ? 1u : 0u) | (sdfk_sel_key(v[1]) <= thr ? 2u : 0u) |
               (sdfk_sel_key(v[2]) <= thr ? 4u : 0u) | (sdfk_sel_key(v[3]) <= thr ? 8u : 0u);
    }
    unsigned m = 0;
// ... 289 lines not shown
    hipLaunchKernelGGL(sdfk_flags_count_kernel, dim3((unsigned)sc.tiles), dim3(SDFK_SEL_THREADS), 0, stream, sc.flags, g, sc.blk);
    hipLaunchKernelGGL(sdfk_select_scan_kernel, dim3(1), dim3(1024), 0, stream, sc.blk, sc.tiles);
    if (d_index && capacity > 0)
        hipLaunchKernelGGL(sdfk_flags_scatter_kernel, dim3((unsigned)sc.tiles), dim3(SDFK_SEL_THREADS), 0, stream, sc.flags, g, sc.blk,
                           reinterpret_cast<long long*>(d_index), sc.blk + sc.tiles, (long long)capacity);
    hipError_t e = hipGetLastError();
    unsigned long long total = 0;
    if (e == hipSuccess) e = hipMemcpyAsync(&total, sc.blk + sc.tiles, sizeof total, hipMemcpyDeviceToHost, stream);
    if (e == hipSuccess) e = hipStreamSynchronize(stream);
    if (e != hipSuccess) return fail(-6, std::string("sdfk_eval_select: ") + hipGetErrorString(e));
    *count = (int64_t)total;
    if (!d_index || total == 0) return 0;
    if ((int64_t)total > capacity) return fail(-1, "sdfk_eval_select: index buffer smaller than the selection");
    return 0;
}
static bool select_tiled(const sdfk_program* p, long long n, long long row_len, int mode) {
    RowGeom rg;
    return !p->sites.empty() && mode != SDFK_MODE_NOCULL && row_len > 0 && rows_geometry(n, row_len, &rg);
}
static int select_prepare(const SelGeom& g, float threshold, void* d_scratch, hipStream_t stream, SelScratch* sc, unsigned* thr) {
    if (!d_scratch || ((uintptr_t)d_scratch & 7)) return fail(-1, "sdfk_eval_select: the scratch must be 8-byte aligned device memory");
    *sc = sel_scratch(d_scratch, g);
    *thr = sdfk_sel_key(threshold);
    if (g.RB == 16) HIPCHK(hipMemsetAsync(sc->flags + sel_words(g), 0, 64 * sizeof(unsigned), stream));
    else HIPCHK(hipMemsetAsync(sc->flags, 0, (size_t)(sel_words(g) + 64) * sizeof(unsigned), stream));
    return 0;
}

extern "C" int sdfk_eval_device_select(sdfk_program* p, const float* d_co, int64_t n, int64_t row_stride, int64_t row_len,
                                       int flat, float threshold, int64_t* d_index, int64_t capacity, int64_t* count,
                                       void* d_scratch, void* stream_, int mode) {
    if (!p || !d_co || !count || n < 0 || capacity < 0) return fail(-1, "sdfk_eval_device_select: bad arguments");
    if (row_stride < n) return fail(-1, "sdfk_eval_device_select: row stride smaller than the point count");
    if (row_len < 0 || (row_len > 0 && n % row_len != 0)) return fail(-1, "sdfk_eval_device_select: the point count is not a multiple of the row length");
    if (p->n_aux > 0) return fail(-1, "sdfk_eval_device_select: staged programs (auxiliary fields) are evaluated to a field first");
    *count = 0;
    if (n == 0) return 0;
    if (mode == SDFK_MODE_AUTO) mode = g_default_mode;
    hipStream_t stream = (hipStream_t)stream_;
    const SelGeom g = sel_geom(n, row_len, select_tiled(p, n, row_len, mode));
    SelScratch sc;
    unsigned thr = 0;
    int rc = select_prepare(g, threshold, d_scratch, stream, &sc, &thr);
    if (rc) return rc;
    if (thr == 0xffffffffu) {
        HIPCHK(hipMemsetAsync(sc.blk, 0, (size_t)(sc.tiles + 1) * sizeof(unsigned long long), stream));
        HIPCHK(hipStreamSynchronize(stream));
        return 0;
    }
    SrcArray a = {d_co, (long long)row_stride};
    const bool vec_ok = aligned16(d_co) && (row_stride % 4 == 0);
    rc = run(p, &a, nullptr, n, nullptr, stream_, mode, vec_ok, g.RB == 16 ? row_len : 0, nullptr, 0, flat != 0, 0, 0, sc.flags, thr);
    if (rc) return rc;
    return flags_finish(g, sc, d_index, capacity, count, stream);
}

extern "C" int sdfk_eval_grid_select(sdfk_program* p, const float* ax0, int64_t n0, const float* ax1, int64_t n1,
                                     const float* ax2, int64_t n2, int64_t start, int64_t n, float threshold,
                                     int64_t* d_index, int64_t capacity, int64_t* count, void* d_scratch, void* stream_,
                                     int mode) {
    if (!p || !count || capacity < 0) return fail(-1, "sdfk_eval_grid_select: bad arguments");
    if (start < 0 || n < 0 || start + n > n0 * n1 * n2) return fail(-1, "sdfk_eval_grid_select: range outside the grid");
    if (p->n_aux > 0) return fail(-1, "sdfk_eval_grid_select: staged programs (auxiliary fields) are evaluated to a field first");
    *count = 0;
    if (n == 0) return 0;
    if (mode == SDFK_MODE_AUTO) mode = g_default_mode;
    hipStream_t stream = (hipStream_t)stream_;
    const long long grow = n2 > 1 ? n2 : n1;
    const bool tiled = start % grow == 0 && select_tiled(p, n, grow, mode);
    const SelGeom g = sel_geom(n, grow, tiled);
    SelScratch sc;
    unsigned thr = 0;
    int rc = select_prepare(g, threshold, d_scratch, stream, &sc, &thr);
    if (rc) return rc;
    if (thr == 0xffffffffu) {
        HIPCHK(hipMemsetAsync(sc.blk, 0, (size_t)(sc.tiles + 1) * sizeof(unsigned long long), stream));
        HIPCHK(hipStreamSynchronize(stream));
        return 0;
    }
    AxisTables t;
    SrcGrid sg;
    rc = upload_axes(ax0, n0, ax1, n1, ax2, n2, stream, &t, &sg, start);
    if (rc) return rc;
    rc = run(p, nullptr, &sg, n, nullptr, stream_, mode, true, 0, nullptr, 0, false, 0, 0, sc.flags, thr);
    if (rc) return rc;
    return flags_finish(g, sc, d_index, capacity, count, stream);
}

extern "C" int sdfk_eval_select_finish(sdfk_program* p, int64_t n, int64_t row_len, int mode, int64_t count, int64_t* d_index,
                                       int64_t capacity, void* d_scratch, void* stream_) {
    if (!p || n < 0 || count < 0 || capacity < 0 || !d_scratch || ((uintptr_t)d_scratch & 7))
        return fail(-1, "sdfk_eval_select_finish: bad arguments");
    if (n == 0 || count == 0) return 0;
    if (!d_index || count > capacity) return fail(-1, "sdfk_eval_select_finish: index buffer smaller than the selection");
    if (mode == SDFK_MODE_AUTO) mode = g_default_mode;
    const SelGeom g = sel_geom(n, row_len, select_tiled(p, n, row_len, mode));
    const SelScratch sc = sel_scratch(d_scratch, g);
    unsigned long long total = 0;
    HIPCHK(hipMemcpy(&total, sc.blk + sc.tiles, sizeof total, hipMemcpyDeviceToHost));
    if ((int64_t)total != count) return fail(-1, "sdfk_eval_select_finish: the scratch does not hold a selection of that size");
    hipLaunchKernelGGL(sdfk_flags_scatter_kernel, dim3((unsigned)sc.tiles), dim3(SDFK_SEL_THREADS), 0, (hipStream_t)stream_,
                       sc.flags, g, sc.blk, reinterpret_cast<long long*>(d_index));
    HIPCHK(hipGetLastError());
    HIPCHK(hipStreamSynchronize((hipStream_t)stream_));
    return 0;
}

#define SDFK_GRAD_BAND 32

static __device__ __forceinline__ float sdfk_diff(float lo, float c, float hi, int pos, int n, bool* central) {
    *central = pos != 0 && pos != n - 1;
    return pos == 0 ? hi - c : (pos == n - 1 ? c - lo : hi - lo);
}
static __device__ __forceinline__ void sdfk_grad_fetch(const float* __restrict__ f, long long q, long long n, float* v) {
    if (q >= 0 && q + 4 <= n) {
        const sdfk_f4u t = *reinterpret_cast<const sdfk_f4u*>(f + q);
        v[0] = t[0]; v[1] = t[1]; v[2] = t[2]; v[3] = t[3];
    } else {
        for (int e = 0; e < 4; ++e) v[e] = (q + e >= 0 && q + e < n) ? f[q + e] : 0.0f;
    }
}

__global__ __launch_bounds__(256) void sdfk_gradient_kernel(const float* __restrict__ f, GridDims d, float* __restrict__ out,
                                                            long long stride, long long n, int ncomp, int normalize, int band,
                                                            unsigned S, unsigned total) {
    const unsigned per = (total + 7) / 8;
    const unsigned L = (sdfk_bx() % 8) * per + sdfk_bx() / 8;
    if (L >= total) return;
    const unsigned s = L % S, t = L / S, i = t % (unsigned)d.n0, b = t / (unsigned)d.n0;
    const long long plane = (long long)d.n1 * d.n2;
    const long long jlo = (long long)b * band, jhi = jlo + band < d.n1 ? jlo + band : d.n1;
    const long long lo = ((long long)i * d.n1 + jlo) * d.n2, hi = ((long long)i * d.n1 + jhi) * d.n2;
    const long long p = ((lo + 3) & ~3ll) + ((long long)s * 256 + sdfk_tx()) * 4;
    if (p >= ((hi + 3) & ~3ll) || p >= n) return;
    long long q = p - (long long)i * plane;
    int ii = (int)i;
    if (q >= plane) {
        q -= plane;
        ++ii;
    }
    int j = plane <= 0xffffffffll ? (int)((unsigned)q / (unsigned)d.n2) : (int)(q / d.n2);
    int k = (int)(q - (long long)j * d.n2);
    float c[4], zl, zr, ylo[4], yhi[4], xlo[4], xhi[4];
    sdfk_grad_fetch(f, p, n, c);
    zl = p > 0 ? f[p - 1] : 0.0f;
    zr = p + 4 < n ? f[p + 4] : 0.0f;
    if (ncomp > 1) {
        sdfk_grad_fetch(f, p - d.n2, n, ylo);
        sdfk_grad_fetch(f, p + d.n2, n, yhi);
    }
    if (ncomp > 2) {
        sdfk_grad_fetch(f, p - plane, n, xlo);
        sdfk_grad_fetch(f, p + plane, n, xhi);
    }
    sdfk_f4 o[3];
    for (int e = 0; e < 4; ++e) {
        bool cx = false, cy = false, cz;
        float gx = ncomp > 2 ? sdfk_diff(xlo[e], c[e], xhi[e], ii, d.n0, &cx) : 0.0f;
        float gy = ncomp > 1 ? sdfk_diff(ylo[e], c[e], yhi[e], j, d.n1, &cy) : 0.0f;
        float gz = sdfk_diff(e ? c[e - 1] : zl, c[e], e < 3 ? c[e + 1] : zr, k, d.n2, &cz);
        if (normalize) {
            sdfk_unit3(gx, gy, gz, cx, cy, cz);
        } else {
            gx = cx ? 0.5f * gx : gx;
            gy = cy ? 0.5f * gy : gy;
            gz = cz ? 0.5f * gz : gz;
        }
// ... 187 lines not shown
```

aegolius_amd/csrc/sdfk_mesh.inc:

```

#include "sdfk_mesh_table.inc"

#define SDFK_MESH_THREADS SDFK_SEL_THREADS

struct MeshGeom {
    long long n;
    long long words;
    long long s[3];
    long long rowlen;
    int d[3];
};

static __device__ __forceinline__ unsigned mesh_bits_at(const unsigned* __restrict__ bits, long long words, long long p) {
    const long long q = p >> 5;
    const unsigned r = (unsigned)p & 31u;
    const unsigned lo = q < words ? bits[q] : 0u;
    const unsigned hi = q + 1 < words ? bits[q + 1] : 0u;
    return r ? (lo >> r) | (hi << (32u - r)) : lo;
}

static __device__ __forceinline__ unsigned mesh_span(long long lo, long long hi) {
    return (unsigned)(((1ull << hi) - 1ull) & ~((1ull << lo) - 1ull));
}

// ... 285 lines not shown
        sc->vblk = reinterpret_cast<unsigned long long*>(c + o_v);
        sc->tblk = reinterpret_cast<unsigned long long*>(c + o_t);
        sc->axes = reinterpret_cast<float*>(c + o_a);
        sc->bits = reinterpret_cast<unsigned*>(c + o_b);
        sc->rec = reinterpret_cast<uint4*>(c + o_r);
        sc->tpre = reinterpret_cast<unsigned*>(c + o_p);
        sc->tiles = tiles;
    }
    return off;
}

static int mesh_geom(int D, const int64_t* dims, MeshGeom* g, const char* who) {
    long long n = 1;
    for (int a = 0; a < D; ++a) {
        if (dims[a] < 2 || dims[a] > 0x3fffffff) return fail(-1, std::string(who) + ": every axis needs 2 to 2^30 points");
        n *= dims[a];
        if (n > (1ll << 46)) return fail(-1, std::string(who) + ": grid too large");
    }
    g->n = n;
    g->words = (n + SDFK_SEL_TILE - 1) / SDFK_SEL_TILE * SDFK_MESH_THREADS;
    g->d[0] = (int)dims[0];
    g->d[1] = (int)dims[1];
    g->d[2] = D == 3 ? (int)dims[2] : 1;
    if (D == 3) {
        g->s[0] = dims[1] * dims[2];
        g->s[1] = dims[2];
        g->s[2] = 1;
        g->rowlen = dims[2];
    } else {
        g->s[0] = dims[1];
        g->s[1] = 1;
        g->s[2] = 0;
        g->rowlen = dims[1];
    }
    if (g->words > 0xffffffffll) return fail(-1, std::string(who) + ": grid too large");
    return 0;
}

static bool mesh_level_ok(float level) { return sdfk_sel_key(level) != 0xffffffffu; }

struct MeshSrc {
    const float* field;
    sdfk_program* prog;
    int mode;
};

static long long mesh_grow(int D, const int64_t* dims) { return D == 3 ? dims[2] : dims[1]; }
static size_t mesh_flag_bytes(int D, const int64_t* dims, long long n) {
    const long long grow = mesh_grow(D, dims);
    if (grow < 32) return 0;
    return (size_t)(sel_words(sel_geom(n, grow, true)) + 64) * sizeof(unsigned);
}
static long long mesh_naxis(int D, const int64_t* dims, bool geo) {
    long long naxis = 0;
    for (int a = 0; a < D; ++a) naxis += dims[a];
    return naxis + (geo && D == 2 ? 1 : 0);
}
static void mesh_scratch(int D, const int64_t* dims, const MeshGeom& g, const MeshSrc& src, void* d_scratch, MeshScratch* sc) {
    mesh_layout(g.n, mesh_naxis(D, dims, src.prog != nullptr), sc, d_scratch, src.prog ? mesh_flag_bytes(D, dims, g.n) : 0);
}

template <int D>
static int mesh_eval_bits(const MeshSrc& src, const int64_t* dims, const MeshGeom& g, const MeshScratch& sc, float level,
                          hipStream_t stream, const char* who) {
    int mode = src.mode == SDFK_MODE_AUTO ? g_default_mode : src.mode;
    const long long grow = mesh_grow(D, dims), rows = g.n / grow;
    const long long slab = std::max(32ll, ((1ll << 32) / grow) & ~31ll);
    if (slab * grow > (1ll << 32)) return fail(-1, std::string(who) + ": rows longer than 2^27 points");
    const bool tiled = select_tiled(src.prog, std::min(slab, rows) * grow, grow, mode);
    const SelGeom sg = sel_geom(g.n, grow, tiled);
    unsigned* flags = tiled ? reinterpret_cast<unsigned*>(sc.rec) : sc.bits;
    if (tiled) HIPCHK(hipMemsetAsync(flags + sel_words(sg), 0, 64 * sizeof(unsigned), stream));
    else HIPCHK(hipMemsetAsync(sc.bits, 0, (size_t)g.words * sizeof(unsigned), stream));
    SrcGrid grid;
    grid.ax0 = sc.axes;
    grid.ax1 = sc.axes + dims[0];
    grid.ax2 = sc.axes + dims[0] + dims[1];
    grid.n1 = (unsigned)dims[1];
    grid.n2 = D == 3 ? (unsigned)dims[2] : 1u;
    for (long long row0 = 0; row0 < rows; row0 += slab) {
        const long long m = std::min(slab, rows - row0) * grow;
        grid.start = row0 * grow;
        unsigned* f0 = flags + (tiled ? row0 * (long long)sg.nchunk : row0 * grow / 32);
        int rc = run(src.prog, nullptr, &grid, m, nullptr, stream, mode, true, 0, nullptr, 0, false, 0, 0, f0, sdfk_sel_key(level));
        if (rc) return rc;
    }
    if (tiled)
        hipLaunchKernelGGL(sdfk_mesh_flags_bits_kernel, dim3((unsigned)(g.words / SDFK_MESH_THREADS)), dim3(SDFK_MESH_THREADS), 0, stream,
                           flags, sg, g.n, sc.bits);
    return 0;
}

template <int D>
static int mesh_count(const MeshSrc& src, const float* const* ax, const int64_t* dims, float level, int64_t* nv, int64_t* nf,
                      void* d_scratch, void* stream_, const char* who) {
    if (!nv || !nf || !(src.field || src.prog) || !d_scratch) return fail(-1, std::string(who) + ": bad arguments");
    *nv = *nf = 0;
    if ((uintptr_t)src.field & 15) return fail(-1, std::string(who) + ": the field must be 16-byte aligned");
    if ((uintptr_t)d_scratch & 255) return fail(-1, std::string(who) + ": the scratch must be 256-byte aligned");
    if (src.prog && src.prog->n_aux > 0)
        return fail(-1, std::string(who) + ": staged programs (auxiliary fields) are evaluated to a field first");
    if (!mesh_level_ok(level)) return fail(-1, std::string(who) + ": the level is NaN");
    MeshGeom g;
    int rc = mesh_geom(D, dims, &g, who);
    if (rc) return rc;
    for (int a = 0; a < D; ++a) {
        if (!ax[a]) return fail(-1, std::string(who) + ": axis table missing");
        for (long long i = 0; i + 1 < dims[a]; ++i)
            if (!(ax[a][i] < ax[a][i + 1])) return fail(-1, std::string(who) + ": axis tables must be strictly increasing");
    }
    MeshScratch sc;
    mesh_scratch(D, dims, g, src, d_scratch, &sc);
    hipStream_t stream = (hipStream_t)stream_;
    long long at = 0;
    for (int a = 0; a < D; ++a) {
        HIPCHK(hipMemcpyAsync(sc.axes + at, ax[a], (size_t)dims[a] * sizeof(float), hipMemcpyHostToDevice, stream));
        at += dims[a];
    }
    const long long nb = sc.tiles;
    if (src.prog) {
        if (D == 2) HIPCHK(hipMemsetAsync(sc.axes + at, 0, sizeof(float), stream));
        rc = mesh_eval_bits<D>(src, dims, g, sc, level, stream, who);
        if (rc) return rc;
    } else {
        hipLaunchKernelGGL(sdfk_select_count_kernel<true>, dim3((unsigned)((nb + SDFK_SEL_TPW - 1) / SDFK_SEL_TPW)), dim3(SDFK_SEL_THREADS),
                           0, stream, src.field, g.n, sdfk_sel_key(level), sc.vblk, sc.bits);
    }
    hipLaunchKernelGGL(sdfk_mesh_count_kernel<D>, dim3((unsigned)nb), dim3(SDFK_MESH_THREADS), 0, stream, sc.bits, g, sc.vblk, sc.tblk,
                       sc.rec, sc.tpre);
    hipLaunchKernelGGL(sdfk_select_scan_kernel, dim3(1), dim3(1024), 0, stream, sc.vblk, nb);
    hipLaunchKernelGGL(sdfk_select_scan_kernel, dim3(1), dim3(1024), 0, stream, sc.tblk, nb);
    hipError_t e = hipGetLastError();
    unsigned long long tot[2] = {0, 0};
    if (e == hipSuccess) e = hipMemcpyAsync(&tot[0], sc.vblk + nb, 8, hipMemcpyDeviceToHost, stream);
    if (e == hipSuccess) e = hipMemcpyAsync(&tot[1], sc.tblk + nb, 8, hipMemcpyDeviceToHost, stream);
    if (e == hipSuccess) e = hipStreamSynchronize(stream);
    if (e != hipSuccess) return fail(-6, std::string(who) + ": " + hipGetErrorString(e));
    *nv = (int64_t)tot[0];
    *nf = (int64_t)tot[1];
    return 0;
}

template <int D, typename IDX>
static void mesh_emit(const MeshSrc& src, const MeshGeom& g, const MeshScratch& sc, float level, float* vout, long long vcap,
                      long long es, void* d_faces, long long fcap, hipStream_t stream) {
    const dim3 grid((unsigned)sc.tiles), block(SDFK_MESH_THREADS);
    if (src.prog)
        hipLaunchKernelGGL((sdfk_mesh_emit_kernel<D, IDX, true>), grid, block, 0, stream, static_cast<const float*>(nullptr), sc.bits, g,
                           sc.axes, level, sc.vblk, sc.tblk, sc.rec, sc.tpre, vout, vcap, es, static_cast<IDX*>(d_faces), fcap);
    else
        hipLaunchKernelGGL((sdfk_mesh_emit_kernel<D, IDX, false>), grid, block, 0, stream, src.field, sc.bits, g, sc.axes, level,
                           sc.vblk, sc.tblk, sc.rec, sc.tpre, vout, vcap, es, static_cast<IDX*>(d_faces), fcap);
}

template <int D>
static int mesh_finish(const MeshSrc& src, const int64_t* dims, float level, int64_t nv, int64_t nf, float* d_vertices,
                       int64_t vcap, void* d_faces, int64_t fcap, int face_bytes, void* d_scratch, void* stream_,
                       const char* who) {
    if (!(src.field || src.prog) || !d_scratch || ((uintptr_t)d_scratch & 255) || nv < 0 || nf < 0 || (face_bytes != 4 && face_bytes != 8))
        return fail(-1, std::string(who) + ": bad arguments");
    if (src.prog && src.prog->n_aux > 0)
        return fail(-1, std::string(who) + ": staged programs (auxiliary fields) are evaluated to a field first");
    if (!mesh_level_ok(level)) return fail(-1, std::string(who) + ": the level is NaN");
    if (nv > vcap || nf > fcap || (nv && !d_vertices) || (nf && !d_faces))
        return fail(-1, std::string(who) + ": output buffers smaller than the mesh");
    if (face_bytes == 4 && nv > 0x7fffffffll) return fail(-1, std::string(who) + ": 32-bit faces need fewer than 2^31 vertices");
    MeshGeom g;
// ... 123 lines not shown
```

include/sdfk.h:

```cpp
#ifndef SDFK_H
#define SDFK_H

#include <stddef.h>
#include <stdint.h>

#ifdef __cplusplus
extern "C" {
#endif

#define SDFK_ABI_VERSION 1

#define SDFK_MODE_AUTO 0
#define SDFK_MODE_INTERPRET 1
#define SDFK_MODE_SPECIALIZED 2
#define SDFK_MODE_NOCULL 3

typedef struct sdfk_program sdfk_program;

int sdfk_abi_version(void);
int sdfk_device_count(void);
const char* sdfk_last_error(void);

sdfk_program* sdfk_program_create(const uint32_t* code, size_t n_instr, const float* params, size_t n_params,
                                  const float* tables, size_t n_tables, int result_reg);
void sdfk_program_destroy(sdfk_program* prog);
int sdfk_program_set_params(sdfk_program* prog, const float* params, size_t n_params);
int sdfk_program_set_cull(sdfk_program* prog, const uint32_t* sites, size_t n_sites, const float* k);
int sdfk_program_chain_members(const sdfk_program* prog);
const char* sdfk_program_source(sdfk_program* prog);
int sdfk_program_compile_check(sdfk_program* prog, size_t* code_size);
#define SDFK_FLAVOUR_PLAIN_ARRAY 0
#define SDFK_FLAVOUR_PLAIN_GRID 1
#define SDFK_FLAVOUR_TILE_ARRAY 2
#define SDFK_FLAVOUR_TILE_GRID 3
#define SDFK_FLAVOUR_TILE_MASK 4
#define SDFK_FLAVOUR_ROWS_ARRAY 5
#define SDFK_FLAVOUR_ROWS_GRID 6
#define SDFK_FLAVOUR_ROWS_MASK 7
#define SDFK_FLAVOUR_ROWS2D_ARRAY 8
#define SDFK_FLAVOUR_ROWS2D_GRID 9
#define SDFK_FLAVOUR_RAYS 10
#define SDFK_FLAVOUR_FLAGS 0x100
#define SDFK_FLAVOUR_XY 0x200
int sdfk_program_compile_flavour(sdfk_program* prog, int flavour, size_t* code_size, double* seconds);
void sdfk_debug_cells_stats(int enable, long long* out8);
void sdfk_debug_rays_stats(int enable, long long* out8);
int sdfk_debug_compile_external(sdfk_program* prog, int flavour, size_t* code_size);
void sdfk_jit_drain(void);
void sdfk_jit_cancel(void);
void sdfk_debug_jit_stats(int64_t* builds, double* seconds);
void sdfk_debug_set_rtc_defs(const char* defs);

int sdfk_eval_device(sdfk_program* prog, const float* d_co, int64_t n, int64_t row_stride, float* d_out,
                     void* stream, int mode);
int sdfk_eval_device_rows(sdfk_program* prog, const float* d_co, int64_t n, int64_t row_stride, int64_t row_len,
                          float* d_out, void* stream, int mode);
int sdfk_eval_device_rows3d(sdfk_program* prog, const float* d_co, int64_t n, int64_t row_stride, int64_t row_len,
                            int64_t plane_rows, int64_t first_row_in_plane, float* d_out, void* stream, int mode);
int sdfk_eval_device_rows2d(sdfk_program* prog, const float* d_co, int64_t n, int64_t row_stride, int64_t row_len,
                            float* d_out, void* stream, int mode);
int sdfk_eval_device_rows2d_xy(sdfk_program* prog, const float* d_xy, int64_t n, int64_t row_stride, int64_t row_len,
                               float* d_out, void* stream, int mode);
int sdfk_eval_host(sdfk_program* prog, const void* co, int co_dtype, int64_t n, int64_t row_stride, float* out,
                   int device, int mode);
int sdfk_eval_host_resident(sdfk_program* prog, const void* co, int co_dtype, int64_t n, int64_t row_stride,
                            float* d_out, int device, int mode);
int sdfk_eval_grid(sdfk_program* prog, const float* ax0, int64_t n0, const float* ax1, int64_t n1, const float* ax2,
                   int64_t n2, int64_t start, int64_t count, float* d_out, void* stream, int mode);
int sdfk_eval_grid_host(sdfk_program* prog, const float* ax0, int64_t n0, const float* ax1, int64_t n1,
                        const float* ax2, int64_t n2, int64_t start, int64_t count, float* out, int device, int mode);
int sdfk_eval_grid_sharded(sdfk_program* prog, const float* ax0, int64_t n0, const float* ax1, int64_t n1,
                           const float* ax2, int64_t n2, int n_shards, const int* devices, float* out, int mode);
int sdfk_eval_grid_sharded_device(sdfk_program* prog, const float* ax0, int64_t n0, const float* ax1, int64_t n1,
                                  const float* ax2, int64_t n2, int n_shards, const int* devices, int gather_device,
                                  float* d_full, int mode);
void sdfk_set_default_mode(int mode);
int sdfk_debug_brick_masks(sdfk_program* prog, const float* d_co, int64_t n, int64_t row_stride, uint64_t* d_masks,
                           void* stream);
int sdfk_debug_row_masks(sdfk_program* prog, const float* d_co, int64_t n, int64_t row_stride, int64_t row_len,
                         uint64_t* d_masks, int64_t* n_bricks, int* brick_rows, void* stream);

int sdfk_eval_device_aux(sdfk_program* prog, const float* d_co, int64_t n, int64_t row_stride, const float* d_aux,
                         int n_aux, int64_t aux_stride, float* d_out, void* stream, int mode);
int sdfk_eval_grid_aux(sdfk_program* prog, const float* ax0, int64_t n0, const float* ax1, int64_t n1, const float* ax2,
                       int64_t n2, int64_t start, int64_t count, const float* d_aux, int n_aux, int64_t aux_stride,
                       float* d_out, void* stream, int mode);
int sdfk_field_min(const float* d_field, int64_t n, float* out_min, void* stream);
int sdfk_grid_box_average(float* d_field, int64_t n0, int64_t n1, int64_t n2, int k0, int k1, int k2, int iterations,
                          void* d_scratch, void* stream);
int sdfk_grid_edge_detect(float* d_field, int64_t n0, int64_t n1, int64_t n2, void* d_scratch, void* stream);
int sdfk_grid_signed(float* d_field, int64_t n0, int64_t n1, int64_t n2, float sep_min, int crop, void* d_scratch,
                     void* stream);
int sdfk_grid_boundary_mask(const float* d_field, int64_t n, float sep_min, unsigned char* d_mask, void* stream);
int sdfk_grid_signed_slab(float* d_slab, int64_t plane0, int64_t planes, const unsigned char* d_mask, int64_t n0, int64_t n1,
                          int64_t n2, int crop, void* d_scratch, void* stream);

size_t sdfk_field_select_scratch(int64_t n);
int sdfk_field_select_finish(int64_t n, int64_t count, int64_t* d_index, int64_t capacity, void* d_scratch, void* stream);

size_t sdfk_eval_select_scratch(int64_t n, int64_t row_len);
int sdfk_eval_device_select(sdfk_program* prog, const float* d_co, int64_t n, int64_t row_stride, int64_t row_len, int flat,
                            float threshold, int64_t* d_index, int64_t capacity, int64_t* count, void* d_scratch,
                            void* stream, int mode);
int sdfk_eval_grid_select(sdfk_program* prog, const float* ax0, int64_t n0, const float* ax1, int64_t n1, const float* ax2,
                          int64_t n2, int64_t start, int64_t count_points, float threshold, int64_t* d_index,
                          int64_t capacity, int64_t* count, void* d_scratch, void* stream, int mode);
int sdfk_eval_select_finish(sdfk_program* prog, int64_t n, int64_t row_len, int mode, int64_t count, int64_t* d_index,
                            int64_t capacity, void* d_scratch, void* stream);
int sdfk_field_select(const float* d_field, int64_t n, float threshold, int64_t* d_index, int64_t capacity,
                      int64_t* count, void* d_scratch, void* stream);
int sdfk_field_gradient(const float* d_field, int64_t n0, int64_t n1, int64_t n2, int ncomp, int normalize,
                        float* d_vec, int64_t row_stride, void* stream);

int sdfk_field_crossings_2d(const float* d_uu, const float* d_ww, int64_t n0, int64_t n1, int64_t n2, double w, double d,
                            double thr, signed char* d_sign, void* stream);
int sdfk_lcwg_eval(int variant, const float* d_uu, const float* d_ww, int64_t n0, int64_t n1, int64_t n2, double w, double d,
                   int sign_kind, double sign_value, const void* d_sign, float* d_vec, int64_t row_stride, void* stream);
int sdfk_lcwg_old_eval(int variant, const float* d_r, int64_t r_stride, const float* d_uu, int64_t n, double w, double d,
                       float* d_vec, int64_t row_stride, void* stream);

typedef struct {
    int32_t op;
    int32_t src[2];
    float imm[4];
} sdfk_vec_instr;
int sdfk_vec_eval_device(const sdfk_vec_instr* prog, int n_instr, const float* d_p, int64_t n, int64_t p_stride,
                         const float* d_streams, int n_streams, int64_t stream_stride, int out_kind, float* d_out,
                         int64_t out_stride, void* stream);
void sdfk_vec_set_interpret(int on);
const char* sdfk_vec_source(const sdfk_vec_instr* prog, int n_instr, int n_streams, int out_kind);
int sdfk_vec_compile_check(const sdfk_vec_instr* prog, int n_instr, int n_streams, int out_kind, size_t* code_size);
int sdfk_vec_eval_host(const sdfk_vec_instr* prog, int n_instr, const void* p, int p_dtype, int64_t n, const float* ax0,
                       int64_t n0, const float* ax1, int64_t n1, const float* ax2, int64_t n2, const float* streams,
                       int n_streams, int out_kind, float* out, int device);
// ... 84 lines not shown
```

Before: 362,400.

## Add lattice row-grid kernel for monotone axes and cache uploaded grid axes

Adds a new 3-D grid row-block kernel that, when the y/z axes are monotone, derives per-tile culling masks from the lattice structure of the grid (per-brick probe folds into shared masks) instead of the previous cell-preparation pass. It also caches the uploaded axis arrays per device, so repeated evaluations with identical axes skip hipMalloc and the host-to-device copies. The new path is default-on, with a legacy build kept behind an env var or define. In exchange it adds host-side comparison and monotonicity scans of the axes, a global cache with user counting, and a more complex kernel whose correctness depends on the lattice geometry checks.

```diff
diff --git a/aegolius_amd/_engine.py b/aegolius_amd/_engine.py
--- a/aegolius_amd/_engine.py
+++ b/aegolius_amd/_engine.py
@@ -16,6 +16,7 @@
  FLAVOUR_ROWS_GRID, FLAVOUR_ROWS_MASK, FLAVOUR_ROWS2D_ARRAY, FLAVOUR_ROWS2D_GRID, FLAVOUR_RAYS) = range(11)
 FLAVOUR_FLAGS = 0x100
 FLAVOUR_XY = 0x200
+FLAVOUR_GRID_LEGACY = 0x400
 
 _c = ctypes
 _vp, _i64, _int, _sz = _c.c_void_p, _c.c_int64, _c.c_int, _c.c_size_t
@@ -38,6 +39,9 @@
     "sdfk_jit_drain": (None, []),
     "sdfk_jit_cancel": (None, []),
     "sdfk_debug_set_rtc_defs": (None, [_c.c_char_p]),
+    "sdfk_debug_flavour_source": (_c.c_char_p, [_vp, _int]),
+    "sdfk_debug_axes_stats": (None, [_c.POINTER(_c.c_longlong), _c.POINTER(_c.c_longlong)]),
+    "sdfk_debug_axes_lookup": (_int, [_vp, _i64, _vp, _i64, _vp, _i64, _c.POINTER(_int)]),
     "sdfk_eval_device": (_int, [_vp, _vp, _i64, _i64, _vp, _vp, _int]),
     "sdfk_eval_device_rows": (_int, [_vp, _vp, _i64, _i64, _i64, _vp, _vp, _int]),
     "sdfk_eval_device_rows2d": (_int, [_vp, _vp, _i64, _i64, _i64, _vp, _vp, _int]),
@@ -372,6 +376,10 @@
         s = lib().sdfk_program_source(self._h)
         return s.decode() if s else None
 
+    def flavour_source(self, flavour):
+        s = lib().sdfk_debug_flavour_source(self._h, int(flavour))
+        return s.decode() if s else None
+
     @property
     def chain_members(self):
         return int(lib().sdfk_program_chain_members(self._h))
diff --git a/aegolius_amd/csrc/sdfk.hip b/aegolius_amd/csrc/sdfk.hip
--- a/aegolius_amd/csrc/sdfk.hip
+++ b/aegolius_amd/csrc/sdfk.hip
@@ -199,6 +199,7 @@
     unsigned long long params_version = 1;
     std::string key;
     std::string source;
+    std::string flavour_text;
     std::vector<sdfk_cullsite> sites;
     std::vector<sdfk_cullsite> sites_all;
     bool chain_mode = false;
@@ -533,6 +534,7 @@
 }
 
 static std::atomic<int> g_twaves_override{0}, g_rwbricks_override{0};
+static std::atomic<bool> g_grid_legacy{[] { const char* e = getenv("SDFK_GRID_LEGACY"); return e && e[0] == '1'; }()};
 static int tile_waves() {
     static int v = [] { const char* e = getenv("SDFK_TWAVES"); int t = e ? atoi(e) : 4; return (t >= 1 && t <= 16) ? t : 4; }();
     const int o = g_twaves_override.load();
@@ -580,6 +582,9 @@
     int yrows;
     unsigned prow, seg0, nb0, bpp;
     unsigned inv_nchunk, inv_bpp;
+};
+struct LatticeArg {
+    unsigned ix0, phase, n1, inv_n1;
 };
 static bool rows_geometry(long long n, long long row_len, RowGeom* g, long long plane_rows = 0, long long plane_phase = 0,
                           bool planes_on = false) {
@@ -733,6 +738,7 @@
     std::lock_guard<std::mutex> lk(g_defs_mu);
     std::string rest;
     int tw = 0, rwb = 0, rwv = 0;
+    bool legacy = false;
     const std::string all = defs ? defs : "";
     size_t pos = 0;
     while (pos < all.size()) {
@@ -743,11 +749,13 @@
         else if (tok.compare(0, 16, "-DSDFK_RWBRICKS=") == 0) rwb = atoi(tok.c_str() + 16);
         else if (tok.compare(0, 14, "-DSDFK_RWAVES=") == 0) rwv = atoi(tok.c_str() + 14);
         else if (!tok.empty()) rest += tok + " ";
+        if (tok.compare(0, 18, "-DSDFK_GRID_LEGACY") == 0) legacy = true;
         pos = sp + 1;
     }
     g_twaves_override = (tw >= 1 && tw <= 16) ? tw : 0;
     g_rwbricks_override = (rwb >= 1 && rwb <= 15) ? rwb : 0;
     g_rwaves_override = (rwv >= 1 && rwv <= 16) ? rwv : 0;
+    g_grid_legacy.store(legacy);
     g_rtc_defs = rest;
 }
 static std::vector<std::string> rtc_options(int geo) {
@@ -1090,10 +1098,12 @@
     return e;
 }
 static std::string flavour_key(const sdfk_program* p, int flavour, int rwb, int with_flags = 0) {
-    return p->key + "|f" + std::to_string(flavour) + ((with_flags & 1) ? "s" : "") + ((with_flags & 2) ? "x" : "") + "|" + rtc_option_key(rwb);
+    return p->key + "|f" + std::to_string(flavour) + ((with_flags & 1) ? "s" : "") + ((with_flags & 2) ? "x" : "") +
+           ((with_flags & 4) ? "l" : "") + "|" + rtc_option_key(rwb);
 }
 static std::string flavour_source(const sdfk_program* p, int flavour, int with_flags = 0) {
     return std::string((with_flags & 1) ? "#define SDFK_FLAGS 1\n" : "") + ((with_flags & 2) ? "#define SDFK_XY 1\n" : "") +
+           ((with_flags & 4) ? "#ifndef SDFK_GRID_LEGACY\n#define SDFK_GRID_LEGACY 1\n#endif\n" : "") +
            sdfk_generate_source(g_ops, SDFK_OP_COUNT, p->code.data(), p->code.size() / 2, p->result_reg, p->sites, flavour,
                                 &p->sites_all);
 }
@@ -1121,7 +1131,8 @@
     int with_flags = 0;
     if (flavour >= 0 && (flavour & SDFK_FLAVOUR_FLAGS)) with_flags |= 1;
     if (flavour >= 0 && (flavour & SDFK_FLAVOUR_XY)) with_flags |= 2;
-    if (flavour >= 0) flavour &= ~(SDFK_FLAVOUR_FLAGS | SDFK_FLAVOUR_XY);
+    if (flavour >= 0 && (flavour & SDFK_FLAVOUR_GRID_LEGACY)) with_flags |= 4;
+    if (flavour >= 0) flavour &= ~(SDFK_FLAVOUR_FLAGS | SDFK_FLAVOUR_XY | SDFK_FLAVOUR_GRID_LEGACY);
     if (flavour < 0 || flavour >= SDFK_FL_COUNT) return fail(-1, "sdfk_program_compile_flavour: unknown flavour");
     if (p->sites.empty() && flavour != SDFK_FL_PLAIN_ARRAY && flavour != SDFK_FL_PLAIN_GRID && flavour != SDFK_FL_RAYS)
         return fail(-2, "sdfk_program_compile_flavour: the program has no cull sites");
@@ -1132,6 +1143,8 @@
     if ((with_flags & 1) && (flavour == SDFK_FL_TILE_ARRAY || flavour == SDFK_FL_TILE_GRID || flavour == SDFK_FL_TILE_MASK ||
                        flavour == SDFK_FL_ROWS_MASK))
         return fail(-2, "sdfk_program_compile_flavour: this flavour has no flag-writing build");
+    if ((with_flags & 4) && flavour != SDFK_FL_ROWS_GRID)
+        return fail(-2, "sdfk_program_compile_flavour: only the 3-D grid row-block flavour has a legacy build");
     const int rwb = rows_geo(p);
     const auto t0 = std::chrono::steady_clock::now();
     std::shared_ptr<CodeObject> e =
@@ -1140,6 +1153,17 @@
     if (code_size) *code_size = e->co.size();
     if (seconds) *seconds = std::chrono::duration<double>(std::chrono::steady_clock::now() - t0).count();
     return 0;
+}
+
+extern "C" const char* sdfk_debug_flavour_source(sdfk_program* p, int flavour) {
+    if (!p || flavour < 0) return nullptr;
+    const int with_flags = ((flavour & SDFK_FLAVOUR_FLAGS) ? 1 : 0) | ((flavour & SDFK_FLAVOUR_XY) ? 2 : 0) |
+                           ((flavour & SDFK_FLAVOUR_GRID_LEGACY) ? 4 : 0);
+    flavour &= ~(SDFK_FLAVOUR_FLAGS | SDFK_FLAVOUR_XY | SDFK_FLAVOUR_GRID_LEGACY);
+    if (flavour >= SDFK_FL_COUNT) return nullptr;
+    std::lock_guard<std::mutex> lk(p->mu);
+    p->flavour_text = flavour_source(p, flavour, with_flags);
+    return p->flavour_text.c_str();
 }
 
 extern "C" int sdfk_debug_compile_external(sdfk_program* p, int flavour, size_t* code_size) {
@@ -1432,7 +1456,7 @@
 static int run(sdfk_program* p, const SrcArray* arr, const SrcGrid* grid, long long n, float* d_out, void* stream_,
                int mode, bool vec_ok, long long row_len = 0, const float* aux = nullptr, long long aux_stride = 0,
                bool flat = false, long long plane_rows = 0, long long plane_phase = 0, unsigned* d_flags = nullptr,
-               unsigned thr_key = 0, bool xy = false) {
+               unsigned thr_key = 0, bool xy = false, bool axes_monotone = false) {
     if (!p) return fail(-1, "null program");
     if (n < 0) return fail(-1, "negative point count");
     if (p->n_aux > 0 && (!aux || aux_stride < n))
@@ -1470,13 +1494,14 @@
     RowGeom rg;
     int flavour = arr ? SDFK_FL_PLAIN_ARRAY : SDFK_FL_PLAIN_GRID;
     const long long grow = grid ? (grid->n2 > 1 ? (long long)grid->n2 : (long long)grid->n1) : 0;
+    bool lattice = grid && grid->n2 > 1 && axes_monotone && !p->chain_mode && !g_grid_legacy.load();
     if (!p->sites.empty() && mode != SDFK_MODE_NOCULL && mode != SDFK_MODE_INTERPRET) {
         if (arr && rows_geometry(n, row_len, &rg, (flat || d_flags) ? 0 : plane_rows, plane_phase, p->chain_mode))
             flavour = (flat || xy) ? SDFK_FL_ROWS2D_ARRAY : SDFK_FL_ROWS_ARRAY;
         else if (arr && vec_ok && !p->chain_mode && !d_flags && !xy) flavour = SDFK_FL_TILE_ARRAY;
         else if (grid && grid->start % grow == 0 &&
                  rows_geometry(n, grow, &rg, (grid->n2 > 1 && !d_flags) ? (long long)grid->n1 : 0,
-                               grid->n2 > 1 ? (grid->start / grow) % (long long)grid->n1 : 0, p->chain_mode))
+                               grid->n2 > 1 ? (grid->start / grow) % (long long)grid->n1 : 0, p->chain_mode || lattice))
             flavour = grid->n2 > 1 ? SDFK_FL_ROWS_GRID : SDFK_FL_ROWS2D_GRID;
         else if (grid && vec_ok && !p->chain_mode && !d_flags) flavour = SDFK_FL_TILE_GRID;
         if (!p->chain_mode && (long long)(p->code.size() / 2) > rows_limit &&
@@ -1486,12 +1511,24 @@
             else if (!d_flags) flavour = is_arr ? SDFK_FL_PLAIN_ARRAY : SDFK_FL_PLAIN_GRID;
         }
     }
+    LatticeArg lat{};
+    if (flavour != SDFK_FL_ROWS_GRID) lattice = false;
+    if (lattice) {
+        const long long n1 = (long long)grid->n1, row0 = grid->start / grow;
+        const bool cut_at_planes = !(rg.nb0 == 0u && (long long)rg.prow >= rg.R);
+        if (!(cut_at_planes || n1 >= 16 || rg.R <= n1) || rg.R + n1 >= 0xffffffffLL || row0 / n1 >= 0x7fffffffLL) lattice = false;
+        lat.ix0 = (unsigned)(row0 / n1);
+        lat.phase = (unsigned)(row0 % n1);
+        lat.n1 = grid->n1;
+        lat.inv_n1 = (unsigned)std::min<unsigned long long>(0xffffffffull, (1ull << 32) / (unsigned long long)n1);
+    }
+    const int grid_legacy = (flavour == SDFK_FL_ROWS_GRID && !p->chain_mode && !lattice) ? 4 : 0;
     std::shared_ptr<SpecModule> sk;
     if (mode != SDFK_MODE_INTERPRET) {
         static const bool async_jit = [] { const char* e = getenv("SDFK_ASYNC_JIT"); return !(e && e[0] == '0'); }();
         const bool wait = mode != SDFK_MODE_AUTO || !p->interp_ok || !async_jit;
         std::string err;
-        sk = get_module(p, device, flavour, wait, &err, (d_flags ? 1 : 0) | (xy ? 2 : 0));
+        sk = get_module(p, device, flavour, wait, &err, (d_flags ? 1 : 0) | (xy ? 2 : 0) | grid_legacy);
         if (sk && sk->failed) {
             if (mode == SDFK_MODE_SPECIALIZED || !p->interp_ok)
                 return fail(-3, "specialised kernel unavailable: " + err);
@@ -1535,7 +1572,7 @@
                     rc = prepare_cells(p, d, sk->fn[1], rg, src, 1, prm, tab, stream, &cells);
                     if (rc) return rc;
                 }
-                void* args[] = {&prm, &tab, &g, &rg, &d_out, &d_flags, &thr_key, &cells};
+                void* args[] = {&prm, &tab, &g, &rg, &d_out, &d_flags, &thr_key, lattice ? (void*)&lat : (void*)&cells};
                 HIPCHK(hipModuleLaunchKernel(sk->fn[0], tiles, 1, 1, rthreads, 1, 1, 0, stream, args, nullptr));
             }
             return 0;
@@ -1754,10 +1791,56 @@
     return 0;
 }
 
+struct AxisCache {
+    std::vector<float> host;
+    int64_t n0 = 0, n1 = 0, n2 = 0;
+    bool monotone = false;
+    float* d = nullptr;
+    size_t cap = 0;
+    int users = 0;
+    std::condition_variable idle;
+};
+static std::mutex g_axes_mu;
+static std::map<int, AxisCache> g_axes;
+static std::atomic<long long> g_axes_uploads{0}, g_axes_hits{0};
+static bool axis_monotone(const float* a, int64_t n) {
+    bool up = true, down = true;
+    for (int64_t i = 0; i < n; ++i) {
+        uint32_t bits;
+        memcpy(&bits, a + i, sizeof bits);
+        if ((bits & 0x7fffffffu) > 0x7f800000u) return false;
+    }
+    for (int64_t i = 1; i < n; ++i) {
+        up = up && a[i - 1] <= a[i];
+        down = down && a[i - 1] >= a[i];
+    }
+    return up || down;
+}
+static bool axes_equal(const AxisCache& c, const float* ax0, int64_t n0, const float* ax1, int64_t n1, const float* ax2, int64_t n2) {
+    return c.n0 == n0 && c.n1 == n1 && c.n2 == n2 && c.host.size() == (size_t)(n0 + n1 + n2) &&
+           memcmp(c.host.data(), ax0, (size_t)n0 * sizeof(float)) == 0 &&
+           memcmp(c.host.data() + n0, ax1, (size_t)n1 * sizeof(float)) == 0 &&
+           memcmp(c.host.data() + n0 + n1, ax2, (size_t)n2 * sizeof(float)) == 0;
+}
+static void axes_keep(AxisCache& c, const float* ax0, int64_t n0, const float* ax1, int64_t n1, const float* ax2, int64_t n2) {
+    c.host.resize((size_t)(n0 + n1 + n2));
+    memcpy(c.host.data(), ax0, (size_t)n0 * sizeof(float));
+    memcpy(c.host.data() + n0, ax1, (size_t)n1 * sizeof(float));
+    memcpy(c.host.data() + n0 + n1, ax2, (size_t)n2 * sizeof(float));
+    c.n0 = n0;
+    c.n1 = n1;
+    c.n2 = n2;
+    c.monotone = axis_monotone(ax1, n1) && axis_monotone(ax2, n2);
+}
 struct AxisTables {
-    float* d = nullptr;
+    AxisCache* c = nullptr;
+    hipStream_t stream = nullptr;
+    bool monotone = false;
     ~AxisTables() {
-        if (d) (void)hipFree(d);
+        if (!c) return;
+        (void)hipStreamSynchronize(stream);
+        std::lock_guard<std::mutex> lk(g_axes_mu);
+        if (--c->users == 0) c->idle.notify_all();
     }
 };
 
@@ -1765,17 +1848,61 @@
                        hipStream_t stream, AxisTables* t, SrcGrid* g, int64_t start) {
     if (!ax0 || !ax1 || !ax2 || n0 < 1 || n1 < 1 || n2 < 1) return fail(-1, "grid axes missing or empty");
     if (n1 > 0x7fffffff || n2 > 0x7fffffff) return fail(-1, "grid axis too long");
-    HIPCHK(hipMalloc(&t->d, (size_t)(n0 + n1 + n2) * sizeof(float)));
-    HIPCHK(hipMemcpyAsync(t->d, ax0, (size_t)n0 * sizeof(float), hipMemcpyHostToDevice, stream));
-    HIPCHK(hipMemcpyAsync(t->d + n0, ax1, (size_t)n1 * sizeof(float), hipMemcpyHostToDevice, stream));
-    HIPCHK(hipMemcpyAsync(t->d + n0 + n1, ax2, (size_t)n2 * sizeof(float), hipMemcpyHostToDevice, stream));
-    g->ax0 = t->d;
-    g->ax1 = t->d + n0;
-    g->ax2 = t->d + n0 + n1;
+    int device = 0;
+    HIPCHK(hipGetDevice(&device));
+    std::unique_lock<std::mutex> lk(g_axes_mu);
+    AxisCache& c = g_axes[device];
+    if (c.d && axes_equal(c, ax0, n0, ax1, n1, ax2, n2)) {
+        ++g_axes_hits;
+    } else {
+        c.idle.wait(lk, [&] { return c.users == 0; });
+        if (!(c.d && axes_equal(c, ax0, n0, ax1, n1, ax2, n2))) {
+            const size_t need = (size_t)(n0 + n1 + n2);
+            if (need > c.cap) {
+                if (c.d) (void)hipFree(c.d);
+                c.d = nullptr;
+                c.cap = 0;
+                c.host.clear();
+                HIPCHK(hipMalloc(&c.d, need * sizeof(float)));
+                c.cap = need;
+            }
+            axes_keep(c, ax0, n0, ax1, n1, ax2, n2);
+            if (hipMemcpyAsync(c.d, c.host.data(), need * sizeof(float), hipMemcpyHostToDevice, stream) != hipSuccess ||
+                hipStreamSynchronize(stream) != hipSuccess) {
+                c.host.clear();
+                (void)hipGetLastError();
+                return fail(-6, "uploading the grid axes failed");
+            }
+            ++g_axes_uploads;
+        } else {
+            ++g_axes_hits;
+        }
+    }
+    ++c.users;
+    t->c = &c;
+    t->stream = stream;
+    t->monotone = c.monotone;
+    g->ax0 = c.d;
+    g->ax1 = c.d + n0;
+    g->ax2 = c.d + n0 + n1;
     g->n1 = (unsigned)n1;
     g->n2 = (unsigned)n2;
     g->start = start;
     return 0;
+}
+extern "C" void sdfk_debug_axes_stats(long long* uploads, long long* hits) {
+    if (uploads) *uploads = g_axes_uploads.load();
+    if (hits) *hits = g_axes_hits.load();
+}
+extern "C" int sdfk_debug_axes_lookup(const float* ax0, int64_t n0, const float* ax1, int64_t n1, const float* ax2, int64_t n2,
+                                      int* monotone) {
+    if (!ax0 || !ax1 || !ax2 || n0 < 1 || n1 < 1 || n2 < 1) return fail(-1, "grid axes missing or empty");
+    std::lock_guard<std::mutex> lk(g_axes_mu);
+    AxisCache& c = g_axes[-1];
+    const bool hit = axes_equal(c, ax0, n0, ax1, n1, ax2, n2);
+    if (!hit) axes_keep(c, ax0, n0, ax1, n1, ax2, n2);
+    if (monotone) *monotone = c.monotone ? 1 : 0;
+    return hit ? 1 : 0;
 }
 
 extern "C" int sdfk_eval_grid(sdfk_program* p, const float* ax0, int64_t n0, const float* ax1, int64_t n1,
@@ -1787,7 +1914,7 @@
     SrcGrid g;
     int rc = upload_axes(ax0, n0, ax1, n1, ax2, n2, (hipStream_t)stream, &t, &g, start);
     if (rc) return rc;
-    rc = run(p, nullptr, &g, count, d_out, stream, mode, aligned16(d_out));
+    rc = run(p, nullptr, &g, count, d_out, stream, mode, aligned16(d_out), 0, nullptr, 0, false, 0, 0, nullptr, 0, false, t.monotone);
     if (rc) return rc;
     HIPCHK(hipStreamSynchronize((hipStream_t)stream));
     return 0;
@@ -1803,7 +1930,7 @@
     SrcGrid g;
     int rc = upload_axes(ax0, n0, ax1, n1, ax2, n2, (hipStream_t)stream, &t, &g, start);
     if (rc) return rc;
-    rc = run(p, nullptr, &g, count, d_out, stream, mode, aligned16(d_out), 0, d_aux, aux_stride);
+    rc = run(p, nullptr, &g, count, d_out, stream, mode, aligned16(d_out), 0, d_aux, aux_stride, false, 0, 0, nullptr, 0, false, t.monotone);
     if (rc) return rc;
     HIPCHK(hipStreamSynchronize((hipStream_t)stream));
     return 0;
@@ -1828,7 +1955,7 @@
     for (int64_t s = 0; s < count && rc == 0; s += chunk) {
         const int64_t m = std::min(chunk, count - s);
         g.start = start + s;
-        rc = run(p, nullptr, &g, m, d_out, nullptr, mode, true);
+        rc = run(p, nullptr, &g, m, d_out, nullptr, mode, true, 0, nullptr, 0, false, 0, 0, nullptr, 0, false, t.monotone);
         if (rc == 0 && hipMemcpy(out + s, d_out, (size_t)m * sizeof(float), hipMemcpyDeviceToHost) != hipSuccess)
             rc = fail(-6, "sdfk_eval_grid_host: device-to-host copy failed");
     }
diff --git a/aegolius_amd/csrc/sdfk_codegen.cpp b/aegolius_amd/csrc/sdfk_codegen.cpp
--- a/aegolius_amd/csrc/sdfk_codegen.cpp
+++ b/aegolius_amd/csrc/sdfk_codegen.cpp
@@ -1700,6 +1700,229 @@
 }
 #endif
 )SDFKR";
+static const char kRowsLattice[] = R"SDFKR(
+struct sdfk_lattice {                           // (host: LatticeArg)
+    unsigned ix0, phase;                        // plane of the slab's first row, that row's index in its plane
+    unsigned n1, inv_n1;                        // rows per plane, floor(2^32 / n1) (sdfk_udiv)
+};
+struct sdfk_latmeta {
+    unsigned long long mask[SDFK_NMASK][SDFK_RNBRICK];   // as sdfk_rowmeta
+    float4 cen[SDFK_NCEN];                      // probe centres (x, y, z, radius): SDFK_NSUB per brick
+    float leafval[SDFK_NLEAF * SDFK_NCEN];      // [leaf][centre]
+};
+struct sdfk_latbrick {                          // wave-uniform
+    long long r0;                               // first row of the block (local to the slab)
+    unsigned nrows;                             // its rows, 0: nothing to do
+    unsigned ix, iy0;                           // plane of row r0 and its index there; row r0 + d has iy0 + d, minus n1 in plane
+                                                // ix + 1 from where that reaches n1 (at most once: host)
+};
+static __device__ __forceinline__ sdfk_latbrick sdfk_lat_brick(const sdfk_rowgeom& g, const sdfk_lattice& t, unsigned rb, bool in) {
+    sdfk_latbrick B;
+    long long rend;
+    unsigned slot, blk;
+    sdfk_block_rows(g, rb, B.r0, rend, &slot, &blk);
+    B.nrows = (in && B.r0 < rend) ? (unsigned)(rend - B.r0 < SDFK_RROWS ? rend - B.r0 : SDFK_RROWS) : 0u;
+    if (g.nb0 == 0u && (long long)g.prow >= g.R) {          // blocks of 16 consecutive rows: one may hold rows of two planes
+        const unsigned a = t.phase + (unsigned)B.r0;
+        const unsigned pl = sdfk_udiv(a, t.n1, t.inv_n1);
+        B.ix = t.ix0 + pl;
+        B.iy0 = a - pl * t.n1;
+    } else if (slot == 0xffffffffu) {                       // blocks cut at planes: the leading partial plane ...
+        B.ix = t.ix0;
+        B.iy0 = t.phase + blk * SDFK_RROWS;
+    } else {                                                // ... and the whole ones
+        B.ix = t.ix0 + (g.seg0 ? 1u : 0u) + slot;
+        B.iy0 = blk * SDFK_RROWS;
+    }
+    return B;
+}
+// Probe centre `sb` of window k of a brick: rows [ra, rb) x points [i0, i0 + ZPS) of the window. Window k of row r
+// starts at point 32 k - (r L mod 32) of the row, so over the rows the points run from 32 k + i0 - max shift to
+// 32 k + i0 + ZPS - 1 - min shift, clamped into the row like the points themselves. The box between the table entries
+// at the first and last index holds every point; centre = its midpoint, radius = the distance to its corners, with the
+// guards of sdfk_rows_bounds (the differences are exact or rounded by half an ulp; 1.0001 is a thousand times that).
+static __device__ __forceinline__ float4 sdfk_lat_centre(const SrcGrid& s, const sdfk_rowgeom& g, const sdfk_lattice& t, long long r0,
+                                                         unsigned nrows, unsigned ix, unsigned iy0, unsigned k, unsigned sb) {
+    constexpr unsigned NZP = SDFK_NSUB > 1 ? 4 : 1, NRP = SDFK_NSUB / NZP, RPS = SDFK_RROWS / NRP, ZPS = SDFK_RZ / NZP;
+    unsigned ra = (sb / NZP) * RPS, rb = ra + RPS;
+    const unsigned i0 = (sb % NZP) * ZPS;
+    if (NRP == 2 && iy0 + nrows > t.n1) {                   // rows of two planes: split where the plane changes, not in the middle
+        const unsigned cut = t.n1 - iy0;                    // (as sdfk_sub_centre: each part is bounded tightly)
+        ra = sb / NZP ? cut : 0u;
+        rb = sb / NZP ? SDFK_RROWS : cut;
+    }
+    rb = rb < nrows ? rb : nrows;                           // rows past the block's end repeat its last row
+    ra = ra < nrows - 1u ? ra : nrows - 1u;
+    rb = rb > ra ? rb : ra + 1u;
+    const unsigned ya = iy0 + ra, yb = iy0 + rb - 1u;
+    float x0, x1, y0, y1;
+    if (yb < t.n1 || ya >= t.n1) {                          // one plane
+        const unsigned w = ya >= t.n1 ? 1u : 0u;
+        x0 = x1 = s.ax0[ix + w];
+        y0 = s.ax1[ya - w * t.n1];
+        y1 = s.ax1[yb - w * t.n1];
+    } else {                                                // two (NRP != 2): both x, the whole extent of y
+        x0 = s.ax0[ix];
+        x1 = s.ax0[ix + 1u];
+        y0 = s.ax1[0];
+        y1 = s.ax1[t.n1 - 1u];
+    }
+    unsigned smin = 31u, smax = 0u;
+#pragma unroll 1
+    for (unsigned r = ra; r < rb; ++r) {
+        const unsigned sh = (unsigned)((r0 + r) * (long long)g.L) & 31u;
+        smin = sh < smin ? sh : smin;
+        smax = sh > smax ? sh : smax;
+    }
+    const int last = (int)g.L - 1;
+    const int za = min(max((int)(32u * k + i0) - (int)smax, 0), last);
+    const int zb = min(max((int)(32u * k + i0 + ZPS - 1u) - (int)smin, 0), last);
+    const float z0 = s.ax2[za], z1 = s.ax2[zb];
+    const float xl = fminf(x0, x1), xh = fmaxf(x0, x1), yl = fminf(y0, y1), yh = fmaxf(y0, y1), zl = fminf(z0, z1), zh = fmaxf(z0, z1);
+    const float cx = 0.5f * (xl + xh), cy = 0.5f * (yl + yh), cz = 0.5f * (zl + zh);
+    const float ex = fmaxf(xh - cx, cx - xl), ey = fmaxf(yh - cy, cy - yl), ez = fmaxf(zh - cz, cz - zl);
+    return make_float4(cx, cy, cz, 1.0001f * sqrtf(ex * ex + ey * ey + ez * ez) + 1e-30f);
+}
+// phases A and B of the tile: probe centres (the lanes of a wave take the sub-bricks of its own bricks), every leaf at
+// every centre, one fold lane per centre; returns this wave's first brick (row block, window)
+static __device__ __forceinline__ void sdfk_lat_prepare(const float* __restrict__ PRM, const float* __restrict__ TAB, const SrcGrid& s,
+                                                        const sdfk_rowgeom& g, const sdfk_lattice& t, sdfk_latmeta* meta,
+                                                        unsigned tile, unsigned& rb0, unsigned& c0) {
+    static_assert(SDFK_RWBRICKS * SDFK_NSUB <= 64, "a lane per probe centre of the wave's bricks");
+    const int lane = sdfk_tx() & 63, wave = __builtin_amdgcn_readfirstlane(sdfk_tx() >> 6);
+    const unsigned q0 = tile * SDFK_RNBRICK + wave * SDFK_RWBRICKS;
+    rb0 = sdfk_udiv(q0, g.nchunk, g.inv_nchunk);
+    c0 = q0 - rb0 * g.nchunk;
+    unsigned rb = rb0, c = c0;
+    long long r0 = 0;
+    unsigned nrows = 0u, ix = 0u, iy0 = 0u, k = 0u;
+#pragma unroll
+    for (int j = 0; j < SDFK_RWBRICKS; ++j) {
+        const sdfk_latbrick B = sdfk_lat_brick(g, t, rb, q0 + j < g.nbricks);
+        if ((unsigned)lane / SDFK_NSUB == (unsigned)j) { r0 = B.r0; nrows = B.nrows; ix = B.ix; iy0 = B.iy0; k = c; }
+        if (++c == g.nchunk) { c = 0; ++rb; }
+    }
+    if (lane < SDFK_RWBRICKS * SDFK_NSUB) {
+        float4 cc = make_float4(0.0f, 0.0f, 0.0f, 1.0f);   // (a dead brick still meets a probe lane: harmless values)
+#ifndef SDFK_ABLATE_BOUNDS
+        if (nrows) cc = sdfk_lat_centre(s, g, t, r0, nrows, ix, iy0, k, (unsigned)lane % SDFK_NSUB);
+#endif
+        meta->cen[wave * (SDFK_RWBRICKS * SDFK_NSUB) + lane] = cc;
+    }
+    if (lane < SDFK_RWBRICKS) {
+#pragma unroll
+        for (int w = 0; w < SDFK_NMASK; ++w) meta->mask[w][wave * SDFK_RWBRICKS + lane] = ~0ull;   // the fold lanes AND their decisions into these
+    }
+    __syncthreads();
+#ifndef SDFK_ABLATE_PROBE
+    sdfk_probe_leaves(meta->cen, meta->leafval, PRM, TAB);
+    __syncthreads();
+    if (sdfk_tx() < SDFK_NCEN && tile * SDFK_RNBRICK + sdfk_tx() / SDFK_NSUB < g.nbricks) {
+        const float4 cc = meta->cen[sdfk_tx()];
+        V3T<float> ctr = {cc.x, cc.y, cc.z};
+        unsigned long long mk[SDFK_NMASK];
+        sdfk_probe_fold(meta->leafval, sdfk_tx(), ctr, cc.w, PRM, mk);
+#pragma unroll
+        for (int w = 0; w < SDFK_NMASK; ++w)
+            __hip_atomic_fetch_and(&meta->mask[w][sdfk_tx() / SDFK_NSUB], mk[w], __ATOMIC_RELAXED, __HIP_MEMORY_SCOPE_WORKGROUP);
+    }
+    __syncthreads();
+#endif
+}
+extern "C" __global__ __launch_bounds__(64 * SDFK_RWAVES) void sdfk_spec_rg(
+    const float* __restrict__ PRM, const float* __restrict__ TAB, SrcGrid s, sdfk_rowgeom g, float* __restrict__ out,
+    unsigned* __restrict__ flags, unsigned thr, sdfk_lattice t) {
+    __shared__ __attribute__((aligned(16))) sdfk_latmeta meta;
+    const int lane = sdfk_tx() & 63, wave = __builtin_amdgcn_readfirstlane(sdfk_tx() >> 6);
+    const int lr = lane / SDFK_RLPR;
+    const int zq = (lane % SDFK_RLPR) * (2 * SDFK_NP);
+    static_assert(SDFK_NP == 4, "a lane takes its eight points as two quads");
+#pragma unroll 1
+  for (unsigned tt = 0; tt < SDFK_RTILES; ++tt) {
+    // (the tile mapping of sdfk_rows_kernel: runs of SDFK_XGROUP consecutive tiles per XCD)
+    const unsigned xg_t = sdfk_bx() / 8;
+    const unsigned tile = (((xg_t / SDFK_XGROUP) * 8 + sdfk_bx() % 8) * SDFK_XGROUP + xg_t % SDFK_XGROUP) * SDFK_RTILES + tt;
+    if (tile * SDFK_RNBRICK >= g.nbricks) break;
+    if (tt) __syncthreads();
+    unsigned rb, c;
+    sdfk_lat_prepare(PRM, TAB, s, g, t, &meta, tile, rb, c);
+    const unsigned q0 = tile * SDFK_RNBRICK + wave * SDFK_RWBRICKS;
+#pragma unroll 1
+    for (int j = 0; j < SDFK_RWBRICKS; ++j) {
+        if (q0 + j >= g.nbricks) break;
+        const int b = wave * SDFK_RWBRICKS + j;
+        const unsigned k = c;
+        const sdfk_latbrick B = sdfk_lat_brick(g, t, rb, true);
+        if (++c == g.nchunk) { c = 0; ++rb; }
+        if (!B.nrows) continue;
+        unsigned mw[2 * SDFK_NMASK];                             // the brick's skip bits as scalar words
+#pragma unroll
+        for (int w = 0; w < SDFK_NMASK; ++w) {
+            const unsigned long long m = meta.mask[w][b];
+            mw[2 * w] = __builtin_amdgcn_readfirstlane((unsigned)m);
+            mw[2 * w + 1] = __builtin_amdgcn_readfirstlane((unsigned)(m >> 32));
+        }
+        const bool interior = sdfk_interior(g.L, k);
+        const bool live_row = (unsigned)lr < B.nrows;
+        const unsigned dr = live_row ? (unsigned)lr : B.nrows - 1u;
+        long long f;                                              // flat index of this lane's first point
+        const int z = sdfk_win_z(B.r0 + dr, g.L, k, zq, &f);      // its index in the row (edge windows: may lie outside)
+        const int last = (int)g.L - 1;
+        const unsigned ya = B.iy0 + dr, yw = ya >= t.n1 ? 1u : 0u;
+        const float x = s.ax0[B.ix + yw], y = s.ax1[ya - yw * t.n1];
+        V3P P[SDFK_NP];
+        f2 res[SDFK_NP];
+        if (interior) {                                           // whole windows lie inside the row
+            const sdfk_f4u za = *reinterpret_cast<const sdfk_f4u*>(s.ax2 + z), zb = *reinterpret_cast<const sdfk_f4u*>(s.ax2 + z + 4);
+            P[0].z = {za.x, za.y};
+            P[1].z = {za.z, za.w};
+            P[2].z = {zb.x, zb.y};
+            P[3].z = {zb.z, zb.w};
+        } else {                                                  // the nearest point of the row instead of what lies outside; never stored
+            SDFK_EACH P[q].z = {s.ax2[min(max(z + 2 * q, 0), last)], s.ax2[min(max(z + 2 * q + 1, 0), last)]};
+        }
+        SDFK_EACH { P[q].x = sp<f2>(x); P[q].y = sp<f2>(y); }
+#ifdef SDFK_ABLATE_EVAL
+        SDFK_EACH res[q] = P[q].z + __builtin_bit_cast(float, mw[0] ^ mw[1] ^ mw[2] ^ mw[3]);
+#else
+        sdfk_rows_culled<true>(x, y, P, mw, PRM, TAB, res);
+#endif
+#ifdef SDFK_FLAGS                                                  // (the flag-writing build: the brick-tiled slots of sdfk_rows_kernel)
+        {
+            unsigned bits = 0u;
+            SDFK_EACH bits |= ((sdfk_sel_key(res[q].x) <= thr ? 1u : 0u) | (sdfk_sel_key(res[q].y) <= thr ? 2u : 0u)) << (2 * q);
+            if (!interior) {
+                unsigned ok = 0u;
+                SDFK_EACH {
+                    if (z + 2 * q >= 0 && z + 2 * q <= last) ok |= 1u << (2 * q);
+                    if (z + 2 * q + 1 >= 0 && z + 2 * q + 1 <= last) ok |= 2u << (2 * q);
+                }
+                bits &= ok;
+            }
+            if (!live_row) bits = 0u;
+            reinterpret_cast<unsigned char*>(flags)[(unsigned long long)(q0 + j) * 64ull + (unsigned)lane] = (unsigned char)bits;
+        }
+#else
+        if (live_row) {
+            float* po = out + f;
+            if (interior) {
+#pragma unroll
+                for (int q = 0; q < SDFK_NP; q += 2) {
+                    sdfk_f4u v = {res[q].x, res[q].y, res[q + 1].x, res[q + 1].y};
+                    __builtin_nontemporal_store(v, reinterpret_cast<sdfk_f4u*>(po + 2 * q));
+                }
+            } else {
+                SDFK_EACH {
+                    if (z + 2 * q >= 0 && z + 2 * q <= last) po[2 * q] = res[q].x;
+                    if (z + 2 * q + 1 >= 0 && z + 2 * q + 1 <= last) po[2 * q + 1] = res[q].y;
+                }
+            }
+        }
+#endif
+    }
+  }
+}
+)SDFKR";
 static const char kRowsMask[] = R"SDFKR(
 // test aid: the skip masks (two 64-bit words per brick: sites 0-31, 32-63; bit 2k = first operand of site k
 // skipped, bit 2k+1 = second) followed by the "uniform rows" flag in a third word
@@ -2703,7 +2926,15 @@
         g.emit_rows_culled(result_reg);
         g.s += kRowsKernel;
         if (all || flavour == SDFK_FL_ROWS_ARRAY || flavour == SDFK_FL_ROWS2D_ARRAY) g.s += kRowsArray;
-        if (all || flavour == SDFK_FL_ROWS_GRID || flavour == SDFK_FL_ROWS2D_GRID) g.s += kRowsGrid;
+        if (flavour == SDFK_FL_ROWS_GRID && g.simt) {
+            g.s += "\n#if defined(SDFK_GRID_LEGACY) || !defined(SDFK_SIMT)\n";
+            g.s += kRowsGrid;
+            g.s += "#else\n";
+            g.s += kRowsLattice;
+            g.s += "#endif\n";
+        } else if (all || flavour == SDFK_FL_ROWS_GRID || flavour == SDFK_FL_ROWS2D_GRID) {
+            g.s += kRowsGrid;
+        }
         if (all || flavour == SDFK_FL_ROWS_MASK) g.s += kRowsMask;
     }
     return g.s;
diff --git a/aegolius_amd/csrc/sdfk_fieldops.inc b/aegolius_amd/csrc/sdfk_fieldops.inc
--- a/aegolius_amd/csrc/sdfk_fieldops.inc
+++ b/aegolius_amd/csrc/sdfk_fieldops.inc
@@ -395,7 +395,7 @@
     SrcGrid sg;
     rc = upload_axes(ax0, n0, ax1, n1, ax2, n2, stream, &t, &sg, start);
     if (rc) return rc;
-    rc = run(p, nullptr, &sg, n, nullptr, stream_, mode, true, 0, nullptr, 0, false, 0, 0, sc.flags, thr);
+    rc = run(p, nullptr, &sg, n, nullptr, stream_, mode, true, 0, nullptr, 0, false, 0, 0, sc.flags, thr, false, t.monotone);
     if (rc) return rc;
     return flags_finish(g, sc, d_index, capacity, count, stream);
 }
diff --git a/aegolius_amd/csrc/sdfk_mesh.inc b/aegolius_amd/csrc/sdfk_mesh.inc
--- a/aegolius_amd/csrc/sdfk_mesh.inc
+++ b/aegolius_amd/csrc/sdfk_mesh.inc
@@ -391,7 +391,7 @@
         const long long m = std::min(slab, rows - row0) * grow;
         grid.start = row0 * grow;
         unsigned* f0 = flags + (tiled ? row0 * (long long)sg.nchunk : row0 * grow / 32);
-        int rc = run(src.prog, nullptr, &grid, m, nullptr, stream, mode, true, 0, nullptr, 0, false, 0, 0, f0, sdfk_sel_key(level));
+        int rc = run(src.prog, nullptr, &grid, m, nullptr, stream, mode, true, 0, nullptr, 0, false, 0, 0, f0, sdfk_sel_key(level), false, true);
         if (rc) return rc;
     }
     if (tiled)
diff --git a/include/sdfk.h b/include/sdfk.h
--- a/include/sdfk.h
+++ b/include/sdfk.h
@@ -42,6 +42,7 @@
 #define SDFK_FLAVOUR_RAYS 10
 #define SDFK_FLAVOUR_FLAGS 0x100
 #define SDFK_FLAVOUR_XY 0x200
+#define SDFK_FLAVOUR_GRID_LEGACY 0x400
 int sdfk_program_compile_flavour(sdfk_program* prog, int flavour, size_t* code_size, double* seconds);
 void sdfk_debug_cells_stats(int enable, long long* out8);
 void sdfk_debug_rays_stats(int enable, long long* out8);
@@ -50,6 +51,10 @@
 void sdfk_jit_cancel(void);
 void sdfk_debug_jit_stats(int64_t* builds, double* seconds);
 void sdfk_debug_set_rtc_defs(const char* defs);
+const char* sdfk_debug_flavour_source(sdfk_program* prog, int flavour);
+void sdfk_debug_axes_stats(long long* uploads, long long* hits);
+int sdfk_debug_axes_lookup(const float* ax0, int64_t n0, const float* ax1, int64_t n1, const float* ax2, int64_t n2,
+                           int* monotone);
 
 int sdfk_eval_device(sdfk_program* prog, const float* d_co, int64_t n, int64_t row_stride, float* d_out,
                      void* stream, int mode);
```

Result: no change. 362,100 (-0.1%).
